# claussss/ubisoft-laforge-daft-exprt

Hardware: AMD Instinct MI355X
Metric: mel frames/sec (fwd+bwd) (higher is better)
Workload: dtype bf16

## Files before the change

include/daft_exprt_hip.h:

```cpp
#ifndef DAFT_EXPRT_HIP_H
#define DAFT_EXPRT_HIP_H

#include <stdint.h>

#ifdef __cplusplus
extern "C" {
#endif

int dx_version(void);
const char* dx_last_error(void);
int dx_prof_enable(int kind, int capacity);
int dx_prof_collect(int kind, int* launches, double* total_ms);

int dx_int_durations(const float* dur, int B, int L, int sampling_rate, int filter_length, int hop_length, int centered,
                     long long* out, long long* totals, int* status);

int dx_pack_dims(int Cout, int Cin, int bf16, int* dims);
int dx_pack_weights(const float* W, void* fwd, void* bwd, int Cout, int Cin, int taps, int bf16, void* stream);
int dx_pack_weights_batched(const void* descs, int n, int bf16, void* stream);
int dx_pack_weights_host(const void* descs, int n, int bf16, void* stream);
int dx_conv_gemm(const void* X, int ldx, const void* Wp, const float* bias, void* Y, int ldy,
                 int B, int N, int Cin, int Cout, int taps, int bf16,
                 int relu, const float* post_scale, const float* post_shift,
                 const void* relu_aux, int ld_aux, int accumulate,
                 const int* lens, int mask_rows, float out_scale, int skip_halo,
                 int x_bf16, int y_bf16, int aux_bf16, const int* rows_exist, void* stream);
int dx_conv_wgrad(const void* dY, int ldy, const void* X, int ldx, float* G,
                  int B, int N, int Cin, int Cout, int taps, const int* lens, int skip_halo,
                  int bf16, int dy_bf16, int x_bf16, float* dbias, void* stream);
typedef struct DxWgradJob {
  const void* dY; const void* X; float* G; float* dbias; const int* lens;
  int ldy, ldx, B, N, Cin, Cout, skip_halo, reserved;
} DxWgradJob;
int dx_conv_wgrad_batched(const void* jobs, int njobs, int taps, int dy_bf16, int x_bf16, void* stream);
int dx_unpack_wgrad(const float* G, float* grad, int Cout, int Cin, int taps, int accumulate, void* stream);
int dx_ff_pair(const void* X, int ldx, const void* Wa, const void* Wb, const float* bias_a, const float* bias_b,
               const void* aux, int ld_aux, void* H, int ldh, float* Y, int ldy,
               int B, int N, int F, int relu_mid, int accumulate, const int* lens, int skip_halo, const int* rows_exist, void* stream);
int dx_ff_pair_ln(const void* X, int ldx, const void* Wa, const void* Wb, const float* bias_a, const float* bias_b, void* H, int ldh, float* Z,
                  int B, int N, int F, const int* lens, int skip_halo, const int* rows_exist,
                  const float* res, const float* ln_w, const float* ln_b, const float* film, int ld_film, float* Yln, float* mean, float* rstd,
                  uint64_t seed_pre, float p_pre, const uint64_t* seed_offset, void* hmask, void* stream);
int dx_ff_pair_ln_qkv(const void* X, int ldx, const void* Wa, const void* Wb, const float* bias_a, const float* bias_b, void* H, int ldh, float* Z,
                      int B, int N, int F, const int* lens, int skip_halo, const int* rows_exist,
                      const float* res, const float* ln_w, const float* ln_b, const float* film, int ld_film, float* Yln, float* mean, float* rstd,
                      uint64_t seed_pre, float p_pre, const uint64_t* seed_offset, const void* Wq, const float* bias_q, void* QKV, void* hmask, void* stream);
int dx_ff_pair_lnbwd(const void* X, int ldx, const void* Wa, const void* Wb, const void* aux, int ld_aux, void* H, int ldh, float* Y,
                     int B, int N, int F, const int* lens, int skip_halo,
                     const float* z, const float* mean, const float* rstd, const float* ln_w, const float* ln_b, void* DG, float* dw, float* db,
                     uint64_t seed_pre, float p_pre, const uint64_t* seed_offset, void* stream);
int dx_ff_block_bwd(const float* dY2, const float* z2, const float* mean2, const float* rstd2, const float* ln2_w, const float* ln2_b,
                    const float* film, int ld_film, void* DG2, float* dw2, float* db2, float* dfilm, int ld_dfilm, uint64_t seed2, float p2,
                    const void* Wa, const void* Wb, const void* aux, int ld_aux, void* H, int ldh, float* Y,
                    int B, int N, int F, const int* lens, int skip_halo,
                    const float* z1, const float* mean1, const float* rstd1, const float* ln1_w, const float* ln1_b, void* DG1, float* dw1, float* db1,
                    uint64_t seed1, float p1, const void* Wout_bwd, void* DATT, const uint64_t* seed_offset, const void* hmask, void* stream);
int dx_colsum(const void* X, int ldx, float* out, long rows, int C, int x_bf16, void* stream);

int dx_length_order(const int* lens, int* order, int B, void* stream);
int dx_attention_fwd(const void* qkv, int ld, const int* lens, void* ctx, int ldc, float* lse,
                     int B, int N, int H, int D, uint64_t seed, const uint64_t* seed_offset, float p_drop, int bf16, int qkv_bf16, int ctx_bf16,
                     const int* order, void* stream);
int dx_attention_proj_ln_fwd(const void* qkv, int ld, const int* lens, void* ctx, int ldc, float* lse, int B, int N, int H, int D,
                             uint64_t seed, const uint64_t* seed_offset, float p_drop,
                             const void* Wpack, const float* proj_bias, float* z, const float* res, const float* w, const float* bias,
                             const float* film, int ld_film, float* y, float* mean, float* rstd, uint64_t seed_pre, float p_pre,
                             void* y_bf16_copy, void* stream);
int dx_attention_bwd(const void* qkv, int ld, const void* ctx, const void* dctx, int ldc, const float* lse, float* delta,
                     const int* lens, void* dqkv, int ldg, int B, int N, int H, int D, uint64_t seed, const uint64_t* seed_offset, float p_drop, int bf16,
                     int qkv_bf16, int dqkv_bf16, int ctx_bf16, const int* order, void* stream);

int dx_ln_fwd(void* a, const void* res, const float* w, const float* bias, const float* film, int ld_film,
              const int* lens, int halo, void* y, float* mean, float* rstd, int B, int N, int C,
              uint64_t seed_pre, float p_pre, uint64_t seed_post, float p_post, const uint64_t* seed_offset, int io_bf16, void* y_bf16_copy,
              void* stream);
int dx_film_affine_fwd(const float* gammas, const float* betas, const float* pm, float* film, int B, int nb, int C, void* stream);
int dx_film_affine_bwd(const void* dfilm_ptrs, const float* gammas, const float* betas, const float* pm, float* dgammas, float* dbetas, float* dpm,
                       int B, int nb, int C, void* stream);
int dx_proj_ln_fwd(const void* X, int ldx, const void* Wpack, const float* proj_bias, float* z, const float* res, const float* w, const float* bias,
                   const float* film, int ld_film, const int* lens, int halo, float* y, float* mean, float* rstd, int B, int N,
                   uint64_t seed_pre, float p_pre, const uint64_t* seed_offset, void* y_bf16_copy, void* stream);
int dx_ln_bwd(const void* dy, const void* z, const float* mean, const float* rstd, const float* w, const float* bias,
              const float* film, int ld_film, const int* lens, int halo, void* dz, void* da, float* dw, float* dbias,
              float* dfilm, int ld_dfilm, int B, int N, int C, int relu_mask,
              uint64_t seed_pre, float p_pre, uint64_t seed_post, float p_post, const uint64_t* seed_offset, int io_bf16, void* dg_bf16_copy,
              void* stream);

int dx_add_pos(const float* x, const long* sym, const float* emb, const float* pe, const int* lens, float* out,
               int B, int N, int D, int pe_rows, void* stream);
int dx_mask_rows(const float* in, const int* lens, float* out, int B, int N, int C, void* stream);
int dx_embedding_bwd(const float* dout, const long* sym, const int* lens, float* demb, int B, int N, int D, void* stream);
int dx_accent_sum(const float* prenet, const float* energy, const float* pitch, const float* we, const float* be,
                  const float* wp, const float* bp, const float* pe, const int* lens, float* out,
                  int B, int N, int D, int pe_rows, void* stream);
int dx_scalar_conv_wgrad(const float* dout, int ldd, const float* rowscale, const float* s0, const float* s1, const int* lens,
                         float* dw0, float* db0, float* dw1, float* db1, int B, int N, int D, void* stream);
int dx_mean_pool(const float* x, const int* lens, float* out, int B, int N, int C, void* stream);
int dx_mean_pool_bwd(const float* dout, const int* lens, float* dx, int B, int N, int C, void* stream);
int dx_transpose(const float* in, float* out, int B, int R, int Cc, int accumulate, void* stream);
int dx_relu_bwd(const float* dy, const float* y, float* out, long n, void* stream);
int dx_channel_affine(const void* x, const float* scale, const float* shift, void* out, long rows, int C, int io_bf16, void* stream);
int dx_l2_normalize(const float* x, float* y, int rows, int C, void* stream);
int dx_cross_entropy(const float* logits, const long* target, float* loss, float* dlogits, int B, int S, void* stream);

int dx_duration_scan(const long* dur_int, float* mu, long* totals, int B, int L, void* stream);
int dx_upsample_prep(const float* enc, const float* dur, const float* energy, const float* pitch,
                     const float* wd, const float* bd, const float* we, const float* be, const float* wp, const float* bp,
                     const float* wr, const float* br, const int* lens, float* xs, float* z, float* sigma,
                     int B, int L, int D, void* stream);
int dx_upsample_fwd(const float* xs, const float* mu, const float* sigma, const int* lens, float* weights, float* xup,
                    int B, int L, int T, int D, void* stream);
int dx_upsample_bwd(const float* dxup, const float* xs, const float* mu, const float* sigma, const float* weights, const int* lens,
                    float* dxs, float* dsigma, int B, int L, int T, int D, void* stream);
int dx_upsample_sym_bwd(const float* dxs_in, const float* dsigma, const float* xs, const float* z, const float* dur, const int* lens,
                        const float* wd, const float* bd, const float* wr, float* dxs_out, float* dz, float* dwr, float* dbr,
                        int B, int L, int D, void* stream);

int dx_mel_stats(const float* mel_pred, const float* mel_target, float* ep, float* et, float* l1sum, float* l2sum,
                 int B, int M, int T, void* stream);
int dx_energy_diff(const float* ep, const float* et, const int* lens, float* des, float* esum, int B, int T, void* stream);
int dx_mel_grad(const float* mel_pred, const float* mel_target, const float* ep, const float* des, const int* lens,
                float c_l1, float c_l2, float c_e, int e_per_total, float* dmel, int B, int M, int T, void* stream);
int dx_loss_finalize(const float* ce, const float* spk_w_dev, float spk_w, const float* dlogits, float* d_spk, int n_logits,
                     const float* pm, float* d_pm, int n_pm, float pmw,
                     const float* l1sum, const float* l2sum, const int* lens, int B, int M, float msw,
                     const float* esum, float ecw, const float* psum, float pcw, float* terms, float* total, float grad_scale, void* stream);
int dx_pitch_mse(const float* pp, int ldp, const float* gt, const int* lens, float* sums, int B, int T, void* stream);
int dx_pitch_grad(const float* pp, int ldp, const float* gt, const int* lens, const float* sums, float scale, float* dpp, int ldd, int B, int T, void* stream);
int dx_pitch_chain_fwd(const float* mel, int B, int M, int T, const int* lens, const void* w0, const void* w1, const void* w2,
                       const float* b0, const float* b1, const float* b2, const float* s0, const float* s1, const float* s2,
                       const float* t0, const float* t1, const float* t2, const float* w3, float b3, float* pp, void* masks, void* stream);
int dx_pitch_chain_bwd(const float* dpp, int B, int M, int T, const int* lens, const void* w0, const void* w1, const void* w2,
                       const float* s0, const float* s1, const float* s2, const float* w3, const void* masks, float* dmel, void* stream);

int dx_condition_prosody(const float* in, float* out, const long* speaker_ids, const float* table, const int* valid,
                         int which, int B, int N, int S, void* stream);
int dx_gather_speaker_rows(const float* emb, const long* speaker_ids, const int* valid, float* out, int B, int E, int S, void* stream);

int dx_sumsq(const float* x, long n, float* out, void* stream);
int dx_adam_step(float* p, const float* g, float* m, float* v, long n, float lr, float beta1, float beta2, float eps,
                 float weight_decay, int step, const float* normsq, float max_norm, float grad_scale, int* skipped,
                 float* norm_out, float* zero_after, void* stream);

#ifdef __cplusplus
}
#endif
#endif
```

ubisoft_laforge_daft_exprt_amd/csrc/dx_f16_names.h:

```cpp
#pragma once
#define dx_accent_sum dx_accent_sum_f16
#define dx_add_pos dx_add_pos_f16
#define dx_attention_bwd dx_attention_bwd_f16
#define dx_attention_fwd dx_attention_fwd_f16
#define dx_attention_proj_ln_fwd dx_attention_proj_ln_fwd_f16
#define dx_channel_affine dx_channel_affine_f16
#define dx_colsum dx_colsum_f16
#define dx_condition_prosody dx_condition_prosody_f16
#define dx_conv_gemm dx_conv_gemm_f16
#define dx_conv_wgrad dx_conv_wgrad_f16
#define dx_conv_wgrad_batched dx_conv_wgrad_batched_f16
#define dx_cross_entropy dx_cross_entropy_f16
#define dx_embedding_bwd dx_embedding_bwd_f16
#define dx_ff_block_bwd dx_ff_block_bwd_f16
#define dx_ff_pair dx_ff_pair_f16
#define dx_ff_pair_ln dx_ff_pair_ln_f16
#define dx_ff_pair_ln_qkv dx_ff_pair_ln_qkv_f16
#define dx_ff_pair_lnbwd dx_ff_pair_lnbwd_f16
#define dx_gather_speaker_rows dx_gather_speaker_rows_f16
#define dx_l2_normalize dx_l2_normalize_f16
#define dx_length_order dx_length_order_f16
#define dx_ln_bwd dx_ln_bwd_f16
#define dx_film_affine_bwd dx_film_affine_bwd_f16
#define dx_film_affine_fwd dx_film_affine_fwd_f16
#define dx_ln_fwd dx_ln_fwd_f16
#define dx_proj_ln_fwd dx_proj_ln_fwd_f16
#define dx_mask_rows dx_mask_rows_f16
#define dx_mean_pool dx_mean_pool_f16
#define dx_mean_pool_bwd dx_mean_pool_bwd_f16
#define dx_pack_dims dx_pack_dims_f16
#define dx_pitch_chain_bwd dx_pitch_chain_bwd_f16
#define dx_pitch_chain_fwd dx_pitch_chain_fwd_f16
#define dx_pack_weights dx_pack_weights_f16
#define dx_pack_weights_batched dx_pack_weights_batched_f16
#define dx_pack_weights_host dx_pack_weights_host_f16
#define dx_relu_bwd dx_relu_bwd_f16
#define dx_scalar_conv_wgrad dx_scalar_conv_wgrad_f16
#define dx_transpose dx_transpose_f16
#define dx_unpack_wgrad dx_unpack_wgrad_f16
```

ubisoft_laforge_daft_exprt_amd/csrc/dx_ffpair.hip:

```cpp
#include "dx_common.h"
#include <algorithm>

namespace {

template <int NJ> struct FP {
  static constexpr int NROW = NJ * 16;
  static constexpr int TOK = NROW - 2;
  static constexpr int HR = NROW + 2;
  static constexpr int IMG = 2 * HR * 128;
  static constexpr int XP = (HR * 16 + 511) / 512;
  static constexpr int RP = (HR + 31) / 32;
};
constexpr int FP_TOK = FP<8>::TOK;

struct FFPairArgs {
  const dx_h16* X; int ldx;
  const dx_h16* Wa; const dx_h16* Wb;
  const float* bias_a; const float* bias_b;
  const dx_h16* aux; int ld_aux;
  dx_h16* H; int ldh;
  float* Y; int ldy;
  int B, N, F;
  int accumulate;
  const int* lens; int skip_halo;
  const int* rows_exist;
  const float* ln_res; const float* ln_w; const float* ln_b; const float* film; int ld_film;
  float* ln_y; float* ln_mean; float* ln_rstd;
  unsigned long long seed_pre; unsigned thresh_pre; float inv_keep_pre; const unsigned long long* seed_offset;
  const dx_h16* q_w; const float* q_bias; dx_h16* q_out;
  const float* lnb_z; const float* lnb_mean; const float* lnb_rstd; const float* lnb_w; const float* lnb_b;
  dx_h16* lnb_dg; float* lnb_dw; float* lnb_db;
  const dx_h16* lnb_wt; dx_h16* lnb_datt;
  const float* lnp_dy; const float* lnp_z; const float* lnp_mean; const float* lnp_rstd; const float* lnp_w; const float* lnp_b;
  const float* lnp_film; int lnp_ld_film;
  dx_h16* lnp_dg; float* lnp_dw; float* lnp_db; float* lnp_dfilm; int lnp_ld_dfilm;
  unsigned long long lnp_seed; unsigned lnp_thresh; float lnp_inv_keep;
  unsigned* hmask;
  unsigned long long* stamps;
};

#ifdef DX_FFPAIR_STAMPS
#define FP_STAMP(K) { if (lane == 0 && wq == 0 && a.stamps) a.stamps[((size_t)blockIdx.x * 2 + role) * 16 + (K)] = __builtin_amdgcn_s_memtime(); }
#else
#define FP_STAMP(K) {}
#endif

__device__ __forceinline__ int fp_lds_off(int row, int slot) { return row * 128 + ((slot ^ (row & 7)) << 4); }

__device__ __forceinline__ uint2 fp_pack4(float a, float b, float c, float d) {
  bf16x4 h;
  h[0] = (dx_h16)a; h[1] = (dx_h16)b; h[2] = (dx_h16)c; h[3] = (dx_h16)d;
  return __builtin_bit_cast(uint2, h);
}

__device__ __forceinline__ int fp_opaque(int x) { asm volatile("" : "+v"(x)); return x; }

__device__ __forceinline__ int fp_wave_sum_i(int v) {
#pragma unroll
  for (int off = 32; off > 0; off >>= 1) v += __shfl_xor(v, off, 64);
  return v;
}

typedef short s16x2 __attribute__((ext_vector_type(2)));

#define FP_MMA(W, X, C) C = DX_MFMA_H16(__builtin_bit_cast(bf16x8, W), __builtin_bit_cast(bf16x8, X), C);

template <bool AUX, bool RELU, int NJ, bool MASK = false>
__global__ __launch_bounds__(512, 2) void ff_pair_kernel(const FFPairArgs a) {
  constexpr int FP_TOK = FP<NJ>::TOK, FP_HR = FP<NJ>::HR, FP_IMG = FP<NJ>::IMG, NROW = FP<NJ>::NROW, XP = FP<NJ>::XP, RP = FP<NJ>::RP;
  extern __shared__ __attribute__((aligned(16))) unsigned char smem[];
  unsigned char* const Xs = smem;
  unsigned char* const Hs0 = smem + FP_IMG;
  unsigned char* const Hs1 = smem + 2 * FP_IMG;
  constexpr int DZ_ROWS = NJ == 8 ? 112 : FP_TOK;
  float* const dzs = a.lnp_w ? reinterpret_cast<float*>(smem + 3 * FP_IMG) : nullptr;

  const int tid = threadIdx.x, lane = tid & 63;
  const int wave = __builtin_amdgcn_readfirstlane(tid >> 6);
  const int role = wave >> 2, wq = wave & 3;
  const int r = lane & 15, g = lane >> 4;
  const int tiles_n = (a.N + FP_TOK - 1) / FP_TOK;
  const int nslices = a.F >> 7;
  FP_STAMP(0)

  const dx_h16* const wbase = role == 0 ? a.Wa + (size_t)(2 * wq) * 4 * 512
                                        : a.Wb + (size_t)(2 * wq) * (a.F >> 5) * 512;
  const unsigned lane16 = lane * 16;
  const int w_tap = role == 0 ? (a.F >> 4) * 4 * 512 : 8 * (a.F >> 5) * 512;
  const int w_i = role == 0 ? 4 * 512 : (a.F >> 5) * 512;
  const int w_slice = role == 0 ? 8 * 4 * 512 : 4 * 512;
  const int total_steps = nslices * 12;
  auto w_ptr = [&](int gs) {
    gs = min(gs, total_steps - 1);
    const int f = fp_opaque(gs / 12), s = gs - f * 12;
    return wbase + (size_t)f * w_slice + (s >> 2) * w_tap + (s & 3) * 512;
  };
  constexpr int RING = NJ == 8 ? 4 : 6;
  f32x4 wr[RING][2];
#define FP_WLOAD(SLOT, GS)                                                                                           \
  {                                                                                                                  \
    const char* p_ = reinterpret_cast<const char*>(w_ptr(GS));                                                       \
    wr[SLOT][0] = *reinterpret_cast<const f32x4*>(p_ + lane16);                                                      \
    wr[SLOT][1] = *reinterpret_cast<const f32x4*>(p_ + (size_t)w_i * 2 + lane16);                                    \
  }

  int b, n0;
  bool live = true;
  if (a.skip_halo >= 0) {
    int nlive = 0;
    int cnt0 = 0, inc0 = 0;
    for (int base = 0; base < a.B; base += 64) {
      const int i = base + lane;
      const int cnt = i < a.B ? min(tiles_n, max(0, (min(a.lens[i] + a.skip_halo, a.N) + FP_TOK - 1) / FP_TOK)) : 0;
      int inc = cnt;
#pragma unroll
      for (int off = 1; off < 64; off <<= 1) { const int v = __shfl_up(inc, off, 64); if (lane >= off) inc += v; }
      if (base == 0) { cnt0 = cnt; inc0 = inc; }
      nlive += __shfl(inc, 63, 64);
    }
    int target = blockIdx.x;
    live = target < nlive;
    if (!live) target -= nlive;
    int run = 0;
    b = 0; n0 = 0;
    for (int base = 0; base < a.B; base += 64) {
      const int i = base + lane;
      int cnt, inc_live;
      if (base == 0) { cnt = cnt0; inc_live = inc0; }
      else {
        cnt = i < a.B ? min(tiles_n, max(0, (min(a.lens[i] + a.skip_halo, a.N) + FP_TOK - 1) / FP_TOK)) : 0;
        inc_live = cnt;
#pragma unroll
        for (int off = 1; off < 64; off <<= 1) { const int v = __shfl_up(inc_live, off, 64); if (lane >= off) inc_live += v; }
      }
      const int rows_here = min(64, a.B - base);
      const int c = live ? cnt : (i < a.B ? tiles_n - cnt : 0);
      const int inc = live ? inc_live : min(lane + 1, rows_here) * tiles_n - inc_live;
      const unsigned long long hit = __ballot(target < run + inc);
      if (hit) {
        const int first = __builtin_ctzll(hit);
        const int excl = __shfl(run + inc - c, first, 64), cnt_b = __shfl(cnt, first, 64);
        b = base + first;
        n0 = (live ? target - excl : cnt_b + (target - excl)) * FP_TOK;
        break;
      }
      run += __shfl(inc, 63, 64);
    }
  } else {
    b = blockIdx.x / tiles_n;
    n0 = (blockIdx.x - b * tiles_n) * FP_TOK;
  }
  FP_STAMP(1)
  b = __builtin_amdgcn_readfirstlane(b);
  n0 = __builtin_amdgcn_readfirstlane(n0);

  if (!live) {
    const int rows = min(FP_TOK, a.N - n0);
    const int hu = a.H ? a.F >> 3 : 0;
    for (int u = tid; u < rows * hu; u += 512) {
      const int row = u / hu, q = u - row * hu;
      *reinterpret_cast<f32x4*>(a.H + ((size_t)b * a.N + n0 + row) * a.ldh + q * 8) = f32x4{0.f, 0.f, 0.f, 0.f};
    }
    if (a.lnb_w)
      for (int u = tid; u < rows * 16; u += 512) {
        const int row = u >> 4, q = u & 15;
        *reinterpret_cast<f32x4*>(a.lnb_dg + ((size_t)b * a.N + n0 + row) * 128 + q * 8) = f32x4{0.f, 0.f, 0.f, 0.f};
        if (a.lnp_w) *reinterpret_cast<f32x4*>(a.lnp_dg + ((size_t)b * a.N + n0 + row) * 128 + q * 8) = f32x4{0.f, 0.f, 0.f, 0.f};
        if (a.lnb_wt) *reinterpret_cast<f32x4*>(a.lnb_datt + ((size_t)b * a.N + n0 + row) * 128 + q * 8) = f32x4{0.f, 0.f, 0.f, 0.f};
      }
    if (a.lnp_w)
      for (int u = tid; u < rows * 32; u += 512) {
        const int row = u >> 5, q = u & 31;
        *reinterpret_cast<f32x4*>(a.Y + ((size_t)b * a.N + n0 + row) * a.ldy + q * 4) = f32x4{0.f, 0.f, 0.f, 0.f};
      }
    if (!a.accumulate)
      for (int u = tid; u < rows * 32; u += 512) {
        const int row = u >> 5, q = u & 31;
        *reinterpret_cast<f32x4*>(a.Y + ((size_t)b * a.N + n0 + row) * a.ldy + q * 4) = f32x4{0.f, 0.f, 0.f, 0.f};
        if (a.ln_w) *reinterpret_cast<f32x4*>(a.ln_y + ((size_t)b * a.N + n0 + row) * 128 + q * 4) = f32x4{0.f, 0.f, 0.f, 0.f};
      }
    if (a.q_w)
      for (int u = tid; u < rows * 48; u += 512) {
        const int row = u / 48, q = u - row * 48;
        *reinterpret_cast<f32x4*>(a.q_out + ((size_t)b * a.N + n0 + row) * 384 + q * 8) = f32x4{0.f, 0.f, 0.f, 0.f};
      }
    return;
  }

  const int NL = a.rows_exist ? a.rows_exist[b] : a.N;
  if (a.lnp_w) {
    const int q = tid & 15;
    const int len_b = a.lens ? a.lens[b] : a.N;
    float wv[8], bv[8], fg[8];
#pragma unroll
    for (int e = 0; e < 8; ++e) {
      wv[e] = a.lnp_w[q * 8 + e]; bv[e] = a.lnp_b[q * 8 + e];
      fg[e] = a.lnp_film ? a.lnp_film[(size_t)b * a.lnp_ld_film + q * 8 + e] : 1.f;
    }
    const unsigned long long seed = a.lnp_seed + (a.seed_offset ? *a.seed_offset : 0ull);
    float gw[8], gb[8], gfg[8], gfb[8];
#pragma unroll
    for (int e = 0; e < 8; ++e) gw[e] = gb[e] = gfg[e] = gfb[e] = 0.f;
    f32x4 dyv[RP][2], zv[RP][2];
    float muv[RP], rsv[RP];
#pragma unroll
    for (int it = 0; it < RP; ++it) {
      const int row = (tid >> 4) + it * 32, n = n0 - 2 + row;
      const bool valid = row < FP_HR && n >= 0 && n < len_b && n < NL;
      const size_t grow = (size_t)b * a.N + n;
#pragma unroll
      for (int hh = 0; hh < 2; ++hh) {
        dyv[it][hh] = valid ? *reinterpret_cast<const f32x4*>(a.lnp_dy + grow * 128 + q * 8 + hh * 4) : f32x4{0.f, 0.f, 0.f, 0.f};
        zv[it][hh] = valid ? *reinterpret_cast<const f32x4*>(a.lnp_z + grow * 128 + q * 8 + hh * 4) : f32x4{0.f, 0.f, 0.f, 0.f};
      }
      muv[it] = valid ? a.lnp_mean[grow] : 0.f;
      rsv[it] = valid ? a.lnp_rstd[grow] : 0.f;
    }
    FP_WLOAD(0, 0) FP_WLOAD(1, 1) FP_WLOAD(2, 2) FP_WLOAD(3, 3)
    if constexpr (RING == 6) { FP_WLOAD(4, 4) FP_WLOAD(5, 5) }
#pragma unroll
    for (int it = 0; it < RP; ++it) {
      const int row = (tid >> 4) + it * 32, n = n0 - 2 + row;
      const bool inb = row < FP_HR && n >= 0 && n < a.N;
      const bool owned = inb && row >= 2 && row < 2 + FP_TOK;
      const bool ownvalid = owned && n < len_b;
      const size_t grow = (size_t)b * a.N + n;
      float dz[8];
      float s1 = 0.f, s2 = 0.f, g[8], xh[8];
#pragma unroll
      for (int e = 0; e < 8; ++e) {
        const float z = zv[it][e >> 2][e & 3];
        float d = dyv[it][e >> 2][e & 3];
        xh[e] = (z - muv[it]) * rsv[it];
        const float ln = xh[e] * wv[e] + bv[e];
        if (ownvalid) { gfg[e] += d * ln; gfb[e] += d; }
        d *= fg[e];
        if (ownvalid) { gw[e] += d * xh[e]; gb[e] += d; }
        g[e] = d * wv[e];
        s1 += g[e]; s2 += g[e] * xh[e];
      }
#pragma unroll
      for (int off = 1; off < 16; off <<= 1) { s1 += __shfl_xor(s1, off, 64); s2 += __shfl_xor(s2, off, 64); }
      s1 *= (1.0f / 128); s2 *= (1.0f / 128);
#pragma unroll
      for (int e = 0; e < 8; ++e) dz[e] = rsv[it] * (g[e] - s1 - xh[e] * s2);
      if (owned) {
        if (dzs && row - 2 < DZ_ROWS) {
          *reinterpret_cast<f32x4*>(dzs + (row - 2) * 128 + q * 8) = f32x4{dz[0], dz[1], dz[2], dz[3]};
          *reinterpret_cast<f32x4*>(dzs + (row - 2) * 128 + q * 8 + 4) = f32x4{dz[4], dz[5], dz[6], dz[7]};
        } else {
          *reinterpret_cast<f32x4*>(a.Y + grow * a.ldy + q * 8) = f32x4{dz[0], dz[1], dz[2], dz[3]};
          *reinterpret_cast<f32x4*>(a.Y + grow * a.ldy + q * 8 + 4) = f32x4{dz[4], dz[5], dz[6], dz[7]};
        }
      }
      if (a.lnp_thresh) {
        float f[8];
        dx_dropout_scale4(seed, (unsigned long long)grow * 128 + q * 8, a.lnp_thresh, a.lnp_inv_keep, f);
        dx_dropout_scale4(seed, (unsigned long long)grow * 128 + q * 8 + 4, a.lnp_thresh, a.lnp_inv_keep, f + 4);
#pragma unroll
        for (int e = 0; e < 8; ++e) dz[e] *= f[e];
      }
      bf16x8 h8;
#pragma unroll
      for (int e = 0; e < 8; ++e) h8[e] = (dx_h16)dz[e];
      const f32x4 hv = __builtin_bit_cast(f32x4, h8);
      if (owned) *reinterpret_cast<f32x4*>(a.lnp_dg + grow * 128 + q * 8) = hv;
      if (row < FP_HR) *reinterpret_cast<f32x4*>(Xs + (q >> 3) * (FP_HR * 128) + fp_lds_off(row, q & 7)) = hv;
    }
#pragma unroll
    for (int e = 0; e < 8; ++e) {
#pragma unroll
      for (int off = 16; off < 64; off <<= 1) {
        gw[e] += __shfl_xor(gw[e], off, 64); gb[e] += __shfl_xor(gb[e], off, 64);
        gfg[e] += __shfl_xor(gfg[e], off, 64); gfb[e] += __shfl_xor(gfb[e], off, 64);
      }
    }
    float* const red = reinterpret_cast<float*>(Hs0);
    if (lane < 16) {
#pragma unroll
      for (int e = 0; e < 8; ++e) {
        red[(wave * 4 + 0) * 128 + q * 8 + e] = gw[e]; red[(wave * 4 + 1) * 128 + q * 8 + e] = gb[e];
        red[(wave * 4 + 2) * 128 + q * 8 + e] = gfg[e]; red[(wave * 4 + 3) * 128 + q * 8 + e] = gfb[e];
      }
    }
    __syncthreads();
    {
      const int quant = tid >> 7, c = tid & 127;
      float t = 0.f;
#pragma unroll
      for (int w8 = 0; w8 < 8; ++w8) t += red[(w8 * 4 + quant) * 128 + c];
      if (t != 0.f) {
        if (quant == 0) atomicAdd(&a.lnp_dw[c], t);
        else if (quant == 1) atomicAdd(&a.lnp_db[c], t);
        else if (a.lnp_dfilm) atomicAdd(&a.lnp_dfilm[(size_t)b * a.lnp_ld_dfilm + (quant == 3 ? 128 : 0) + c], t);
      }
    }
    __syncthreads();
    if (tid < 64) {
      const int img = tid >> 5, rr = NROW + ((tid >> 4) & 1), qq = tid & 15;
      *reinterpret_cast<f32x4*>((img ? Hs1 : Hs0) + (qq >> 3) * (FP_HR * 128) + fp_lds_off(rr, qq & 7)) = f32x4{0.f, 0.f, 0.f, 0.f};
    }
  } else
  {
    f32x4 xr[XP];
#pragma unroll
    for (int it = 0; it < XP; ++it) {
      const int u = tid + it * 512;
      const int row = u >> 4, q = u & 15;
      const int n = n0 - 2 + row;
      f32x4 v = f32x4{0.f, 0.f, 0.f, 0.f};
      if (u < FP_HR * 16 && n >= 0 && n < NL) v = *reinterpret_cast<const f32x4*>(a.X + ((size_t)b * a.N + n) * a.ldx + q * 8);
      xr[it] = v;
    }
    FP_WLOAD(0, 0) FP_WLOAD(1, 1) FP_WLOAD(2, 2) FP_WLOAD(3, 3)
    if constexpr (RING == 6) { FP_WLOAD(4, 4) FP_WLOAD(5, 5) }
    if (tid < 64) {
      const int img = tid >> 5, rr = NROW + ((tid >> 4) & 1), q = tid & 15;
      *reinterpret_cast<f32x4*>((img ? Hs1 : Hs0) + (q >> 3) * (FP_HR * 128) + fp_lds_off(rr, q & 7)) = f32x4{0.f, 0.f, 0.f, 0.f};
    }
#pragma unroll
    for (int it = 0; it < XP; ++it) {
      const int u = tid + it * 512;
      const int row = u >> 4, q = u & 15;
      if (u < FP_HR * 16) *reinterpret_cast<f32x4*>(Xs + (q >> 3) * (FP_HR * 128) + fp_lds_off(row, q & 7)) = xr[it];
    }
  }
  __syncthreads();
  FP_STAMP(2)

  int foff[3][2];
#pragma unroll
  for (int t = 0; t < 3; ++t)
#pragma unroll
    for (int hh = 0; hh < 2; ++hh) foff[t][hh] = fp_lds_off(r + t, hh * 4 + g);
  const int len_cols = min(FP_TOK, a.N - n0);
  const int h_rows = a.H ? len_cols : 0;

#define FP_CO_RD(K, IMGC)                                                                                            \
  {                                                                                                                  \
    const int u_ = fp_opaque(tid) + NROW * 8 + (K) * 256;        \
    const int row_ = u_ >> 4, q_ = u_ & 15;                                                                          \
    cpv = *reinterpret_cast<const f32x4*>((IMGC) + (q_ >> 3) * (FP_HR * 128) + fp_lds_off(min(row_, NROW - 1) + 1, q_ & 7)); \
  }
#define FP_CO_ST(K, F0C)                                                                                             \
  {                                                                                                                  \
    const int u_ = fp_opaque(tid) + NROW * 8 + (K) * 256;                                                            \
    const int row_ = u_ >> 4, q_ = u_ & 15;                                                                          \
    if (row_ < h_rows) *reinterpret_cast<f32x4*>(a.H + ((size_t)b * a.N + n0 + row_) * a.ldh + (F0C) + q_ * 8) = cpv; \
  }
#define FP_COPY_OUT_CONS(IMGC, F0C)                                                                                  \
  {                                                                                                                  \
    f32x4 cv_[NJ / 2];                                                                                               \
    const int t_ = fp_opaque(tid) - 256;                        \
    _Pragma("unroll") for (int k = 0; k < NJ / 2; ++k) {                                                                  \
      const int u_ = t_ + k * 256;                                                                                   \
      cv_[k] = *reinterpret_cast<const f32x4*>((IMGC) + ((u_ & 15) >> 3) * (FP_HR * 128) + fp_lds_off((u_ >> 4) + 1, u_ & 7)); \
    }                                                                                                                \
    _Pragma("unroll") for (int k = 0; k < NJ / 2; ++k) {                                                             \
      const int u_ = t_ + k * 256;                                                                                   \
      const int row_ = u_ >> 4, q_ = u_ & 15;                                                                        \
      if (row_ < h_rows) *reinterpret_cast<f32x4*>(a.H + ((size_t)b * a.N + n0 + row_) * a.ldh + (F0C) + q_ * 8) = cv_[k]; \
    }                                                                                                                \
  }

#define FP_RD8(DST, IMG, S)                                                                                          \
  {                                                                                                                  \
    const unsigned char* const bp_ = (IMG) + (((S) & 3) >> 1) * (FP_HR * 128) + foff[((S) >> 2) % 3][(S) & 1];       \
    _Pragma("unroll") for (int j = 0; j < NJ; ++j) DST[j] = *reinterpret_cast<const float4*>(bp_ + j * 2048);        \
  }
#define FP_STEP(CUR, NXT, IMG, GS0, S, AUXPF, FRESH, CO, IMGC, F0C)                                                  \
  {                                                                                                                  \
    if ((S) + 1 < 12) FP_RD8(NXT, IMG, (S) + 1)                                                                      \
    if ((CO) && (S) < NJ && ((S) & 1) == 0) FP_CO_RD((S) >> 1, IMGC)                                                 \
    __builtin_amdgcn_sched_barrier(0);                                                                               \
    const f32x4 w0 = wr[(S) % RING][0], w1 = wr[(S) % RING][1];                                                      \
    if ((FRESH) && (S) == 0) {                                   \
      _Pragma("unroll") for (int j = 0; j < NJ; ++j) { acc[0][j] = bv0; FP_MMA(w0, CUR[j], acc[0][j]) }              \
      _Pragma("unroll") for (int j = 0; j < NJ; ++j) { acc[1][j] = bv1; FP_MMA(w1, CUR[j], acc[1][j]) }              \
    } else {                                                                                                         \
      _Pragma("unroll") for (int j = 0; j < NJ; ++j) { FP_MMA(w0, CUR[j], acc[0][j]) }                               \
      _Pragma("unroll") for (int j = 0; j < NJ; ++j) { FP_MMA(w1, CUR[j], acc[1][j]) }                               \
    }                                                                                                                \
    FP_WLOAD((S) % RING, (GS0) + (S) + RING)                                                                         \
    if ((CO) && (S) < NJ && ((S) & 1) == 1) FP_CO_ST((S) >> 1, F0C)                                                  \
    if ((S) == 8) { AUXPF }                                                                                          \
    __builtin_amdgcn_sched_barrier(0);                                                                               \
  }
#define FP_SLICE_STEPS(IMG, GS0, AUXPF, FR, CO, IMGC, F0C)                                                           \
  {                                                                                                                  \
    float4 xa[NJ], xb[NJ];                                                                                           \
    f32x4 cpv;                                                                                                       \
    FP_RD8(xa, IMG, 0)                                                                                               \
    FP_STEP(xa, xb, IMG, GS0, 0, AUXPF, FR, CO, IMGC, F0C) FP_STEP(xb, xa, IMG, GS0, 1, AUXPF, FR, CO, IMGC, F0C)    \
    FP_STEP(xa, xb, IMG, GS0, 2, AUXPF, FR, CO, IMGC, F0C) FP_STEP(xb, xa, IMG, GS0, 3, AUXPF, FR, CO, IMGC, F0C)    \
    FP_STEP(xa, xb, IMG, GS0, 4, AUXPF, FR, CO, IMGC, F0C) FP_STEP(xb, xa, IMG, GS0, 5, AUXPF, FR, CO, IMGC, F0C)    \
    FP_STEP(xa, xb, IMG, GS0, 6, AUXPF, FR, CO, IMGC, F0C) FP_STEP(xb, xa, IMG, GS0, 7, AUXPF, FR, CO, IMGC, F0C)    \
    FP_STEP(xa, xb, IMG, GS0, 8, AUXPF, FR, CO, IMGC, F0C) FP_STEP(xb, xa, IMG, GS0, 9, AUXPF, FR, CO, IMGC, F0C)    \
    FP_STEP(xa, xb, IMG, GS0, 10, AUXPF, FR, CO, IMGC, F0C) FP_STEP(xb, xa, IMG, GS0, 11, AUXPF, FR, CO, IMGC, F0C)  \
  }

  unsigned char* const stage = smem;
  if (role == 0) {
    f32x4 acc[2][NJ];
    const bool edge = n0 == 0 || n0 + FP_TOK >= NL;
    const int tile_lin = b * tiles_n + n0 / FP_TOK;
#define FP_PRODUCE(F_, COFLAG)                                                                                       \
    {                                                                                                                \
      const int f0 = (F_) << 7;                                                                                      \
                                   \
      const f32x4 bv0 = a.bias_a ? *reinterpret_cast<const f32x4*>(a.bias_a + f0 + 32 * wq + 4 * g) : f32x4{0.f, 0.f, 0.f, 0.f};      \
      const f32x4 bv1 = a.bias_a ? *reinterpret_cast<const f32x4*>(a.bias_a + f0 + 32 * wq + 16 + 4 * g) : f32x4{0.f, 0.f, 0.f, 0.f}; \
      bf16x4 av[2][MASK ? 1 : NJ];                                                                                   \
      unsigned mw[2] = {0u, 0u};                                                                                     \
      FP_SLICE_STEPS(Xs, (F_) * 12,                                                                                  \
        if constexpr (AUX) {                                                                                         \
          if constexpr (MASK) {                                                                                      \
            const unsigned* mp_ = a.hmask + ((((size_t)tile_lin * nslices + (f0 >> 7)) * 4 + wq) * 2) * 64 + fp_opaque(lane); \
            mw[0] = mp_[0]; mw[1] = mp_[64];                                                                         \
          } else {                                                                                                   \
          const int r2_ = fp_opaque(r);                                                                              \
          const int g2_ = fp_opaque(g);                                                                              \
          _Pragma("unroll") for (int i = 0; i < 2; ++i)                                                              \
            _Pragma("unroll") for (int j = 0; j < NJ; ++j) {                                                         \
              const int n = min(max(n0 - 1 + 16 * j + r2_, 0), a.N - 1);                                             \
              av[i][j] = *reinterpret_cast<const bf16x4*>(a.aux + ((size_t)b * a.N + n) * a.ld_aux + f0 + 32 * wq + 16 * i + 4 * g2_); \
            }                                                                                                        \
          }                                                                                                          \
        }, true, COFLAG, ((((F_) - 1) & 1) ? Hs1 : Hs0), ((F_) - 1) * 128)                                           \
      unsigned char* const out = ((F_) & 1) ? Hs1 : Hs0;                                                             \
      const int r_ = fp_opaque(r);                                                                                   \
      const int g_ = fp_opaque(g);                                                                                   \
      _Pragma("unroll") for (int i = 0; i < 2; ++i) {                                                                \
        const int c = 32 * wq + 16 * i + 4 * g_;                                                                     \
        unsigned char* const orow = out + (c >> 6) * (FP_HR * 128) + fp_lds_off(r_, (c & 63) >> 3) + ((g_ & 1) << 3); \
        unsigned sw_ = 0u;                                                  \
        const unsigned mwi_ = mw[i];                                                                                 \
        _Pragma("unroll") for (int j = 0; j < NJ; ++j) {                                                             \
          f32x4 v = acc[i][j];                                                                                       \
          if constexpr (AUX) {                                                                                       \
            if constexpr (MASK) {                                                                                    \
               \
              _Pragma("unroll") for (int e = 0; e < 4; ++e) {                                                        \
                const float ve_ = v[e];                                                                              \
                const unsigned ke_ = __float_as_uint(ve_) & (unsigned)__builtin_amdgcn_sbfe((int)mwi_, NJ * 4 - 1 - (j * 4 + e), 1); \
                v[e] = __uint_as_float(ke_);                                                                         \
              }                                                                                                      \
            } else {                                                                                                 \
              _Pragma("unroll") for (int e = 0; e < 4; ++e) if (!((float)av[i][j][e] > 0.f)) v[e] = 0.f;             \
            }                                                                                                        \
          }                                                                                                          \
          if (edge) { const int n = n0 - 1 + 16 * j + r_; if (n < 0 || n >= NL) v = f32x4{0.f, 0.f, 0.f, 0.f}; }    \
          if constexpr (RELU) {                                                                                      \
             \
            if (a.hmask) {                                                                                           \
              _Pragma("unroll") for (int e = 0; e < 4; ++e) {                                                        \
                const float ve_ = v[e];                                                                              \
                sw_ = __builtin_amdgcn_alignbit(sw_, __float_as_uint(ve_) - 1u, 31);                                 \
              }                                                                                                      \
            }                                                                                                        \
          }                                                                                                          \
          uint2 pk = fp_pack4(v[0], v[1], v[2], v[3]);                                                               \
          if constexpr (RELU) {                                                                                      \
             \
            pk.x = __builtin_bit_cast(unsigned, __builtin_elementwise_max(__builtin_bit_cast(s16x2, pk.x), s16x2{0, 0})); \
            pk.y = __builtin_bit_cast(unsigned, __builtin_elementwise_max(__builtin_bit_cast(s16x2, pk.y), s16x2{0, 0})); \
          }                                                                                                          \
          *reinterpret_cast<uint2*>(orow + j * 2048) = pk;                                                           \
        }                                                                                                            \
        if constexpr (RELU) {                                        \
          if (a.hmask) a.hmask[((((size_t)tile_lin * nslices + (f0 >> 7)) * 4 + wq) * 2 + i) * 64 + fp_opaque(lane)] = ~sw_; \
        }                                                                                                            \
      }                                                                                                              \
    }
    FP_PRODUCE(0, false)
    __syncthreads();
    FP_STAMP(3)
    for (int it = 1; it < nslices; ++it) {
      if (it == 4) FP_STAMP(12)
      FP_PRODUCE(it, true)
      if (it == 4) FP_STAMP(14)
      __syncthreads();
      FP_STAMP(3 + it)
    }
    {
      const unsigned char* const imgc = ((nslices - 1) & 1) ? Hs1 : Hs0;
      f32x4 cpv;
#pragma unroll
      for (int k = 0; k < NJ / 2; ++k) { FP_CO_RD(k, imgc) FP_CO_ST(k, (nslices - 1) << 7) }
    }
    __syncthreads();
    FP_STAMP(3 + nslices)
#undef FP_PRODUCE
  } else {
    f32x4 acc[2][NJ];
    const f32x4 bv0 = f32x4{0.f, 0.f, 0.f, 0.f}, bv1 = bv0;
#pragma unroll
    for (int i = 0; i < 2; ++i)
#pragma unroll
      for (int j = 0; j < NJ; ++j) acc[i][j] = f32x4{0.f, 0.f, 0.f, 0.f};
    __syncthreads();
    FP_STAMP(3)
    for (int it = 1; it <= nslices; ++it) {
      if (it == 4) FP_STAMP(12)
      const int f = it - 1;
      const unsigned char* const img = (f & 1) ? Hs1 : Hs0;
      FP_COPY_OUT_CONS(img, f << 7)
      FP_SLICE_STEPS(img, f * 12, , false, false, img, 0)
      if (it == 4) FP_STAMP(13)
      __syncthreads();
      FP_STAMP(3 + it)
    }
#pragma unroll
    for (int i = 0; i < 2; ++i) {
      const int co = 32 * wq + 16 * i + 4 * g;
      const f32x4 bv = a.bias_b ? *reinterpret_cast<const f32x4*>(a.bias_b + co) : f32x4{0.f, 0.f, 0.f, 0.f};
#pragma unroll
      for (int j = 0; j < NJ; ++j) {
        const int q = 16 * j + r;
        *reinterpret_cast<f32x4*>(stage + q * 512 + (((co >> 2) ^ (q & 15)) << 4)) = acc[i][j] + bv;
      }
    }
  }
#undef FP_SLICE_STEPS
#undef FP_STEP
#undef FP_RD8
#undef FP_COPY_OUT_CONS
#undef FP_CO_RD
#undef FP_CO_ST

  __syncthreads();
  if (a.ln_w) {
    const int s = tid & 31;
    const f32x4 wv = *reinterpret_cast<const f32x4*>(a.ln_w + s * 4), bv = *reinterpret_cast<const f32x4*>(a.ln_b + s * 4);
    f32x4 fg = f32x4{1.f, 1.f, 1.f, 1.f}, fb = f32x4{0.f, 0.f, 0.f, 0.f};
    if (a.film) {
      fg = *reinterpret_cast<const f32x4*>(a.film + (size_t)b * a.ld_film + s * 4);
      fb = *reinterpret_cast<const f32x4*>(a.film + (size_t)b * a.ld_film + 128 + s * 4);
    }
    const int len_b = a.lens ? a.lens[b] : a.N;
    const unsigned long long seed = a.seed_pre + (a.seed_offset ? *a.seed_offset : 0ull);
    bf16x8 qa[3][4];
    if (a.q_w) {
#pragma unroll
      for (int i = 0; i < 3; ++i)
#pragma unroll
        for (int ks = 0; ks < 4; ++ks) qa[i][ks] = *reinterpret_cast<const bf16x8*>(a.q_w + (size_t)((wave * 3 + i) * 4 + ks) * 512 + lane * 8);
    }
    f32x4 resv[NJ];
#pragma unroll
    for (int k = 0; k < NJ; ++k) {
      const int row = (tid >> 5) + k * 16, n = n0 + row;
      resv[k] = (row < len_cols && n < len_b) ? *reinterpret_cast<const f32x4*>(a.ln_res + ((size_t)b * a.N + n) * 128 + s * 4) : f32x4{0.f, 0.f, 0.f, 0.f};
    }
#pragma unroll
    for (int k = 0; k < NJ; ++k) {
      const int row = (tid >> 5) + k * 16, n = n0 + row;
      const bool inb = row < len_cols, valid = inb && n < len_b;
      const size_t grow = (size_t)b * a.N + n;
      f32x4 z = f32x4{0.f, 0.f, 0.f, 0.f};
      if (valid) {
        z = *reinterpret_cast<const f32x4*>(stage + row * 512 + ((s ^ (row & 15)) << 4));
        if (a.thresh_pre) {
          float f[4];
          dx_dropout_scale4(seed, (unsigned long long)grow * 128 + s * 4, a.thresh_pre, a.inv_keep_pre, f);
          z[0] *= f[0]; z[1] *= f[1]; z[2] *= f[2]; z[3] *= f[3];
        }
        z += resv[k];
      }
      if (inb) *reinterpret_cast<f32x4*>(a.Y + grow * a.ldy + s * 4) = z;
      float sum = (z[0] + z[1]) + (z[2] + z[3]);
#pragma unroll
      for (int off = 1; off < 32; off <<= 1) sum += __shfl_xor(sum, off, 64);
      const float mu = sum * (1.0f / 128);
      const f32x4 d = z - mu;
      float q = (d[0] * d[0] + d[1] * d[1]) + (d[2] * d[2] + d[3] * d[3]);
#pragma unroll
      for (int off = 1; off < 32; off <<= 1) q += __shfl_xor(q, off, 64);
      const float rs = 1.0f / sqrtf(q * (1.0f / 128) + 1e-5f);
      if (inb && s == 0) { a.ln_mean[grow] = valid ? mu : 0.f; a.ln_rstd[grow] = valid ? rs : 0.f; }
      f32x4 y = d * rs * wv + bv;
      if (a.film) y = fg * y + fb;
      if (!valid) y = f32x4{0.f, 0.f, 0.f, 0.f};
      if (inb) *reinterpret_cast<f32x4*>(a.ln_y + grow * 128 + s * 4) = y;
      if (a.q_w) {
        bf16x4 h4;
        h4[0] = (dx_h16)y[0]; h4[1] = (dx_h16)y[1]; h4[2] = (dx_h16)y[2]; h4[3] = (dx_h16)y[3];
        *reinterpret_cast<bf16x4*>(stage + row * 512 + (((s >> 1) ^ (row & 15)) << 4) + ((s & 1) << 3)) = h4;
      }
    }
    if (a.q_w) {
      __syncthreads();
      f32x4 qb[3];
#pragma unroll
      for (int i = 0; i < 3; ++i) qb[i] = *reinterpret_cast<const f32x4*>(a.q_bias + (wave * 3 + i) * 16 + g * 4);
#pragma unroll 2
      for (int j = 0; j < NJ; ++j) {
        const int row = j * 16 + r;
        bf16x8 xb[4];
#pragma unroll
        for (int ks = 0; ks < 4; ++ks) xb[ks] = *reinterpret_cast<const bf16x8*>(stage + row * 512 + (((ks * 4 + g) ^ (row & 15)) << 4));
        f32x4 acc[3];
#pragma unroll
        for (int i = 0; i < 3; ++i) acc[i] = qb[i];
#pragma unroll
        for (int ks = 0; ks < 4; ++ks)
#pragma unroll
          for (int i = 0; i < 3; ++i) acc[i] = DX_MFMA_H16(qa[i][ks], xb[ks], acc[i]);
        if (row < len_cols) {
          dx_h16* const orow = a.q_out + ((size_t)b * a.N + n0 + row) * 384 + wave * 48 + g * 4;
#pragma unroll
          for (int i = 0; i < 3; ++i) {
            bf16x4 o4;
            o4[0] = (dx_h16)acc[i][0]; o4[1] = (dx_h16)acc[i][1]; o4[2] = (dx_h16)acc[i][2]; o4[3] = (dx_h16)acc[i][3];
            *reinterpret_cast<bf16x4*>(orow + i * 16) = o4;
          }
        }
      }
    }
  } else if (a.lnb_w) {
    const int s = tid & 31;
    const f32x4 wv = *reinterpret_cast<const f32x4*>(a.lnb_w + s * 4), bv = *reinterpret_cast<const f32x4*>(a.lnb_b + s * 4);
    (void)bv;
    const int len_b = a.lens ? a.lens[b] : a.N;
    const unsigned long long seed = a.seed_pre + (a.seed_offset ? *a.seed_offset : 0ull);
    f32x4 oldv[NJ], zv[NJ];
    float muv[NJ], rsv[NJ];
#pragma unroll
    for (int k = 0; k < NJ; ++k) {
      const int row = (tid >> 5) + k * 16, n = n0 + row;
      const bool valid = row < len_cols && n < len_b;
      const size_t grow = (size_t)b * a.N + n;
      if (dzs && row < DZ_ROWS) oldv[k] = valid ? *reinterpret_cast<const f32x4*>(dzs + row * 128 + s * 4) : f32x4{0.f, 0.f, 0.f, 0.f};
      else oldv[k] = valid ? *reinterpret_cast<const f32x4*>(a.Y + grow * a.ldy + s * 4) : f32x4{0.f, 0.f, 0.f, 0.f};
      zv[k] = valid ? *reinterpret_cast<const f32x4*>(a.lnb_z + grow * 128 + s * 4) : f32x4{0.f, 0.f, 0.f, 0.f};
      muv[k] = valid ? a.lnb_mean[grow] : 0.f;
      rsv[k] = valid ? a.lnb_rstd[grow] : 0.f;
    }
    f32x4 gw = f32x4{0.f, 0.f, 0.f, 0.f}, gb = gw;
#pragma unroll
    for (int k = 0; k < NJ; ++k) {
      const int row = (tid >> 5) + k * 16, n = n0 + row;
      const bool inb = row < len_cols, valid = inb && n < len_b;
      const size_t grow = (size_t)b * a.N + n;
      f32x4 d = f32x4{0.f, 0.f, 0.f, 0.f};
      if (valid) d = *reinterpret_cast<const f32x4*>(stage + row * 512 + ((s ^ (row & 15)) << 4)) + oldv[k];
      const f32x4 xh = (zv[k] - muv[k]) * rsv[k];
      gw += d * xh; gb += d;
      const f32x4 g = d * wv;
      float s1 = (g[0] + g[1]) + (g[2] + g[3]);
      const f32x4 gx = g * xh;
      float s2 = (gx[0] + gx[1]) + (gx[2] + gx[3]);
#pragma unroll
      for (int off = 1; off < 32; off <<= 1) { s1 += __shfl_xor(s1, off, 64); s2 += __shfl_xor(s2, off, 64); }
      s1 *= (1.0f / 128); s2 *= (1.0f / 128);
      f32x4 dz = (g - s1 - xh * s2) * rsv[k];
      if (!inb) continue;
      *reinterpret_cast<f32x4*>(a.Y + grow * a.ldy + s * 4) = dz;
      if (a.thresh_pre) {
        float f[4];
        dx_dropout_scale4(seed, (unsigned long long)grow * 128 + s * 4, a.thresh_pre, a.inv_keep_pre, f);
        dz[0] *= f[0]; dz[1] *= f[1]; dz[2] *= f[2]; dz[3] *= f[3];
      }
      bf16x4 h4;
      h4[0] = (dx_h16)dz[0]; h4[1] = (dx_h16)dz[1]; h4[2] = (dx_h16)dz[2]; h4[3] = (dx_h16)dz[3];
      *reinterpret_cast<bf16x4*>(a.lnb_dg + grow * 128 + s * 4) = h4;
      if (a.lnb_wt) *reinterpret_cast<bf16x4*>(stage + row * 512 + (((s >> 1) ^ (row & 15)) << 4) + ((s & 1) << 3)) = h4;
    }
    if (a.lnb_wt) {
#pragma unroll
      for (int k = 0; k < NJ; ++k) {
        const int row = (tid >> 5) + k * 16;
        if (row >= len_cols) *reinterpret_cast<uint2*>(stage + row * 512 + (((s >> 1) ^ (row & 15)) << 4) + ((s & 1) << 3)) = make_uint2(0u, 0u);
      }
    }
    float* const red = reinterpret_cast<float*>(smem + NROW * 512);
    *reinterpret_cast<f32x4*>(red + (tid >> 5) * 128 + s * 4) = gw;
    *reinterpret_cast<f32x4*>(red + 2048 + (tid >> 5) * 128 + s * 4) = gb;
    __syncthreads();
    if (tid < 256) {
      const float* src = red + (tid >> 7) * 2048 + (tid & 127);
      float t = 0.f;
#pragma unroll
      for (int q = 0; q < 16; ++q) t += src[q * 128];
      if (t != 0.f) atomicAdd((tid >> 7) ? &a.lnb_db[tid & 127] : &a.lnb_dw[tid & 127], t);
    }
    if (a.lnb_wt) {
      constexpr int CB = NJ;
      const int rb = wave % NJ, cb0 = (wave / NJ) * CB;
      const int row = rb * 16 + r;
      bf16x8 xb[4];
#pragma unroll
      for (int ks = 0; ks < 4; ++ks) xb[ks] = *reinterpret_cast<const bf16x8*>(stage + row * 512 + (((ks * 4 + g) ^ (row & 15)) << 4));
      f32x4 acc[CB];
#pragma unroll
      for (int i = 0; i < CB; ++i) acc[i] = f32x4{0.f, 0.f, 0.f, 0.f};
#pragma unroll
      for (int ks = 0; ks < 4; ++ks) {
        bf16x8 wa[CB];
#pragma unroll
        for (int i = 0; i < CB; ++i) wa[i] = *reinterpret_cast<const bf16x8*>(a.lnb_wt + (size_t)((cb0 + i) * 4 + ks) * 512 + lane * 8);
#pragma unroll
        for (int i = 0; i < CB; ++i) acc[i] = DX_MFMA_H16(wa[i], xb[ks], acc[i]);
      }
      if (row < len_cols) {
        dx_h16* const orow = a.lnb_datt + ((size_t)b * a.N + n0 + row) * 128 + cb0 * 16 + g * 4;
#pragma unroll
        for (int i = 0; i < CB; ++i) {
          bf16x4 o4;
          o4[0] = (dx_h16)acc[i][0]; o4[1] = (dx_h16)acc[i][1]; o4[2] = (dx_h16)acc[i][2]; o4[3] = (dx_h16)acc[i][3];
          *reinterpret_cast<bf16x4*>(orow + i * 16) = o4;
        }
      }
    }
  } else {
    f32x4 old[NJ];
    if (a.accumulate) {
#pragma unroll
      for (int k = 0; k < NJ; ++k) {
        const int u = tid + k * 512;
        const int row = min(u >> 5, len_cols - 1), s = u & 31;
        old[k] = *reinterpret_cast<const f32x4*>(a.Y + ((size_t)b * a.N + n0 + row) * a.ldy + s * 4);
      }
    }
#pragma unroll
    for (int k = 0; k < NJ; ++k) {
      const int u = tid + k * 512;
      const int row = u >> 5, s = u & 31;
      f32x4 v = *reinterpret_cast<const f32x4*>(stage + row * 512 + ((s ^ (row & 15)) << 4));
      if (a.accumulate) v += old[k];
      if (row < len_cols) *reinterpret_cast<f32x4*>(a.Y + ((size_t)b * a.N + n0 + row) * a.ldy + s * 4) = v;
    }
  }
  FP_STAMP(15)
#undef FP_WLOAD
}

#undef FP_MMA

}

#ifdef DX_FFPAIR_STAMPS
static unsigned long long* g_ffpair_stamps = nullptr;
extern "C" void dx_ff_pair_set_stamps(unsigned long long* p) { g_ffpair_stamps = p; }
#endif

extern "C" {

static int ff_pair_launch(const void* X, int ldx, const void* Wa, const void* Wb, const float* bias_a, const float* bias_b,
                          const void* aux, int ld_aux, void* H, int ldh, float* Y, int ldy,
                          int B, int N, int F, int relu_mid, int accumulate, const int* lens, int skip_halo, const int* rows_exist,
                          const float* ln_res, const float* ln_w, const float* ln_b, const float* film, int ld_film,
                          float* ln_y, float* ln_mean, float* ln_rstd, unsigned long long seed_pre, float p_pre, const unsigned long long* seed_offset,
                          const float* lnb_z, const float* lnb_mean, const float* lnb_rstd, const float* lnb_w, const float* lnb_b,
                          void* lnb_dg, float* lnb_dw, float* lnb_db, const FFPairArgs* prologue, void* stream, unsigned* hmask = nullptr) {
  DX_REQUIRE((X || prologue) && Wa && Wb && Y, "dx_ff_pair: null pointer");
  DX_REQUIRE(H || (relu_mid && !lnb_w), "dx_ff_pair: only the forward pair may omit the mid-activation output H");
  if (ln_w) {
    DX_REQUIRE(relu_mid && !accumulate && lens && skip_halo >= 0 && ldy == 128, "dx_ff_pair_ln: forward pair, no accumulate, lens, dense Z");
    DX_REQUIRE(ln_res && ln_b && ln_y && ln_mean && ln_rstd, "dx_ff_pair_ln: null pointer");
    DX_REQUIRE(!film || ld_film >= 256, "dx_ff_pair_ln: ld_film too small");
    DX_REQUIRE(p_pre >= 0.f && p_pre < 1.f, "dx_ff_pair_ln: dropout p out of range");
  }
  if (lnb_w) {
    DX_REQUIRE(aux && accumulate && lens && skip_halo >= 0 && ldy == 128 && !ln_w, "dx_ff_pair_lnbwd: input-gradient pair accumulating onto a dense Y, lens required");
    DX_REQUIRE(lnb_z && lnb_mean && lnb_rstd && lnb_b && lnb_dg && lnb_dw && lnb_db, "dx_ff_pair_lnbwd: null pointer");
    DX_REQUIRE(p_pre >= 0.f && p_pre < 1.f && ((uintptr_t)lnb_dg % 16) == 0, "dx_ff_pair_lnbwd: bad dropout p or alignment");
  }
  DX_REQUIRE(B > 0 && N > 0 && F >= 128 && (F % 128) == 0, "dx_ff_pair: bad dims B=%d N=%d F=%d (F must be a multiple of 128)", B, N, F);
  DX_REQUIRE(ldx >= 128 && (ldx % 8) == 0 && ldh >= F && (ldh % 8) == 0 && ldy >= 128 && (ldy % 4) == 0, "dx_ff_pair: bad leading dimensions");
  DX_REQUIRE(!aux || (ld_aux >= F && (ld_aux % 4) == 0), "dx_ff_pair: bad ld_aux");
  DX_REQUIRE((aux != nullptr) != (relu_mid != 0), "dx_ff_pair: exactly one of relu_mid (forward) and aux (backward) must be given");
  DX_REQUIRE(skip_halo < 0 || lens, "dx_ff_pair: skip_halo needs lens");
  if (prologue && prologue->q_w) {
    DX_REQUIRE(ln_w && prologue->q_bias && prologue->q_out && ((uintptr_t)prologue->q_w % 16) == 0 && ((uintptr_t)prologue->q_out % 16) == 0,
               "dx_ff_pair_ln_qkv: needs the LayerNorm epilogue, a bias and 16-byte aligned pointers");
  } else if (prologue) {
    DX_REQUIRE(lnb_w && prologue->lnp_dy && prologue->lnp_z && prologue->lnp_mean && prologue->lnp_rstd && prologue->lnp_w && prologue->lnp_b &&
               prologue->lnp_dg && prologue->lnp_dw && prologue->lnp_db, "dx_ff_block_bwd: null pointer");
    DX_REQUIRE((prologue->lnp_film == nullptr) == (prologue->lnp_dfilm == nullptr), "dx_ff_block_bwd: film and dfilm must come together");
    DX_REQUIRE(((uintptr_t)prologue->lnp_dy % 16) == 0 && ((uintptr_t)prologue->lnp_z % 16) == 0 && ((uintptr_t)prologue->lnp_dg % 16) == 0,
               "dx_ff_block_bwd: pointers must be 16-byte aligned");
  }
  DX_REQUIRE(((uintptr_t)X % 16) == 0 && ((uintptr_t)Wa % 16) == 0 && ((uintptr_t)Wb % 16) == 0 && ((uintptr_t)H % 16) == 0 &&
             ((uintptr_t)Y % 16) == 0 && ((uintptr_t)aux % 8) == 0, "dx_ff_pair: pointers must be 16-byte aligned");
  FFPairArgs a{(const dx_h16*)X, ldx, (const dx_h16*)Wa, (const dx_h16*)Wb, bias_a, bias_b, (const dx_h16*)aux, ld_aux,
               (dx_h16*)H, ldh, Y, ldy, B, N, F, accumulate, lens, skip_halo, rows_exist,
               ln_res, ln_w, ln_b, film, ld_film, ln_y, ln_mean, ln_rstd, seed_pre, (unsigned)lrintf(p_pre * 65536.f), 1.f / (1.f - p_pre), seed_offset,
               nullptr, nullptr, nullptr,
               lnb_z, lnb_mean, lnb_rstd, lnb_w, lnb_b, (dx_h16*)lnb_dg, lnb_dw, lnb_db};
  if (prologue && prologue->q_w) { a.q_w = prologue->q_w; a.q_bias = prologue->q_bias; a.q_out = prologue->q_out; }
  if (prologue && prologue->lnp_dy) {
    a.lnp_dy = prologue->lnp_dy; a.lnp_z = prologue->lnp_z; a.lnp_mean = prologue->lnp_mean; a.lnp_rstd = prologue->lnp_rstd;
    a.lnp_w = prologue->lnp_w; a.lnp_b = prologue->lnp_b; a.lnp_film = prologue->lnp_film; a.lnp_ld_film = prologue->lnp_ld_film;
    a.lnp_dg = prologue->lnp_dg; a.lnp_dw = prologue->lnp_dw; a.lnp_db = prologue->lnp_db; a.lnp_dfilm = prologue->lnp_dfilm;
    a.lnp_ld_dfilm = prologue->lnp_ld_dfilm; a.lnp_seed = prologue->lnp_seed; a.lnp_thresh = prologue->lnp_thresh; a.lnp_inv_keep = prologue->lnp_inv_keep;
    a.lnb_wt = prologue->lnb_wt; a.lnb_datt = prologue->lnb_datt;
  }
#ifdef DX_FFPAIR_STAMPS
  a.stamps = g_ffpair_stamps;
#endif
  constexpr int DZ8 = 112 * 512, DZ4 = FP<4>::TOK * 512;
  const int lds8 = 3 * FP<8>::IMG + (a.lnp_w ? DZ8 : 0), lds4 = 3 * FP<4>::IMG + (a.lnp_w ? DZ4 : 0);
  static bool configured = false;
  if (!configured) {
    hipFuncSetAttribute(reinterpret_cast<const void*>(&ff_pair_kernel<true, false, 8>), hipFuncAttributeMaxDynamicSharedMemorySize, 3 * FP<8>::IMG + DZ8);
    hipFuncSetAttribute(reinterpret_cast<const void*>(&ff_pair_kernel<true, false, 8, true>), hipFuncAttributeMaxDynamicSharedMemorySize, 3 * FP<8>::IMG + DZ8);
    hipFuncSetAttribute(reinterpret_cast<const void*>(&ff_pair_kernel<true, false, 4, true>), hipFuncAttributeMaxDynamicSharedMemorySize, 3 * FP<4>::IMG + DZ4);
    hipFuncSetAttribute(reinterpret_cast<const void*>(&ff_pair_kernel<false, true, 8>), hipFuncAttributeMaxDynamicSharedMemorySize, 3 * FP<8>::IMG);
    hipFuncSetAttribute(reinterpret_cast<const void*>(&ff_pair_kernel<true, false, 4>), hipFuncAttributeMaxDynamicSharedMemorySize, 3 * FP<4>::IMG + DZ4);
    hipFuncSetAttribute(reinterpret_cast<const void*>(&ff_pair_kernel<false, true, 4>), hipFuncAttributeMaxDynamicSharedMemorySize, 3 * FP<4>::IMG);
    configured = true;
  }
  a.hmask = hmask;
  const int nj = B * dx_cdiv(N, FP<8>::TOK) >= 96 ? 8 : 4;
  hipStream_t s = (hipStream_t)stream;
  dx_prof_begin(DX_PROF_CONV_GEMM, s);
  if (nj == 8) {
    if (aux && hmask) hipLaunchKernelGGL((ff_pair_kernel<true, false, 8, true>), dim3(B * dx_cdiv(N, FP<8>::TOK)), dim3(512), lds8, s, a);
    else if (aux) hipLaunchKernelGGL((ff_pair_kernel<true, false, 8>), dim3(B * dx_cdiv(N, FP<8>::TOK)), dim3(512), lds8, s, a);
    else hipLaunchKernelGGL((ff_pair_kernel<false, true, 8>), dim3(B * dx_cdiv(N, FP<8>::TOK)), dim3(512), 3 * FP<8>::IMG, s, a);
  } else {
    if (aux && hmask) hipLaunchKernelGGL((ff_pair_kernel<true, false, 4, true>), dim3(B * dx_cdiv(N, FP<4>::TOK)), dim3(512), lds4, s, a);
    else if (aux) hipLaunchKernelGGL((ff_pair_kernel<true, false, 4>), dim3(B * dx_cdiv(N, FP<4>::TOK)), dim3(512), lds4, s, a);
    else hipLaunchKernelGGL((ff_pair_kernel<false, true, 4>), dim3(B * dx_cdiv(N, FP<4>::TOK)), dim3(512), 3 * FP<4>::IMG, s, a);
  }
  dx_prof_end(DX_PROF_CONV_GEMM, s);
  DX_LAUNCH_CHECK("dx_ff_pair");
  return DX_OK;
}

int dx_ff_pair(const void* X, int ldx, const void* Wa, const void* Wb, const float* bias_a, const float* bias_b,
               const void* aux, int ld_aux, void* H, int ldh, float* Y, int ldy,
               int B, int N, int F, int relu_mid, int accumulate, const int* lens, int skip_halo, const int* rows_exist, void* stream) {
  return ff_pair_launch(X, ldx, Wa, Wb, bias_a, bias_b, aux, ld_aux, H, ldh, Y, ldy, B, N, F, relu_mid, accumulate, lens, skip_halo, rows_exist,
                        nullptr, nullptr, nullptr, nullptr, 0, nullptr, nullptr, nullptr, 0ull, 0.f, nullptr,
                        nullptr, nullptr, nullptr, nullptr, nullptr, nullptr, nullptr, nullptr, nullptr, stream);
}

int dx_ff_pair_ln(const void* X, int ldx, const void* Wa, const void* Wb, const float* bias_a, const float* bias_b, void* H, int ldh, float* Z,
                  int B, int N, int F, const int* lens, int skip_halo, const int* rows_exist,
                  const float* res, const float* ln_w, const float* ln_b, const float* film, int ld_film, float* Yln, float* mean, float* rstd,
                  uint64_t seed_pre, float p_pre, const uint64_t* seed_offset, void* hmask, void* stream) {
  DX_REQUIRE(ln_w != nullptr, "dx_ff_pair_ln: null pointer");
  return ff_pair_launch(X, ldx, Wa, Wb, bias_a, bias_b, nullptr, 0, H, ldh, Z, 128, B, N, F, 1, 0, lens, skip_halo, rows_exist,
                        res, ln_w, ln_b, film, ld_film, Yln, mean, rstd, (unsigned long long)seed_pre, p_pre, (const unsigned long long*)seed_offset,
                        nullptr, nullptr, nullptr, nullptr, nullptr, nullptr, nullptr, nullptr, nullptr, stream, (unsigned*)hmask);
}

int dx_ff_pair_ln_qkv(const void* X, int ldx, const void* Wa, const void* Wb, const float* bias_a, const float* bias_b, void* H, int ldh, float* Z,
                      int B, int N, int F, const int* lens, int skip_halo, const int* rows_exist,
                      const float* res, const float* ln_w, const float* ln_b, const float* film, int ld_film, float* Yln, float* mean, float* rstd,
                      uint64_t seed_pre, float p_pre, const uint64_t* seed_offset, const void* Wq, const float* bias_q, void* QKV, void* hmask, void* stream) {
  DX_REQUIRE(ln_w != nullptr && Wq != nullptr, "dx_ff_pair_ln_qkv: null pointer");
  FFPairArgs ext{};
  ext.q_w = (const dx_h16*)Wq; ext.q_bias = bias_q; ext.q_out = (dx_h16*)QKV;
  return ff_pair_launch(X, ldx, Wa, Wb, bias_a, bias_b, nullptr, 0, H, ldh, Z, 128, B, N, F, 1, 0, lens, skip_halo, rows_exist,
                        res, ln_w, ln_b, film, ld_film, Yln, mean, rstd, (unsigned long long)seed_pre, p_pre, (const unsigned long long*)seed_offset,
                        nullptr, nullptr, nullptr, nullptr, nullptr, nullptr, nullptr, nullptr, &ext, stream, (unsigned*)hmask);
}

int dx_ff_pair_lnbwd(const void* X, int ldx, const void* Wa, const void* Wb, const void* aux, int ld_aux, void* H, int ldh, float* Y,
                     int B, int N, int F, const int* lens, int skip_halo,
                     const float* z, const float* mean, const float* rstd, const float* ln_w, const float* ln_b, void* DG, float* dw, float* db,
                     uint64_t seed_pre, float p_pre, const uint64_t* seed_offset, void* stream) {
  DX_REQUIRE(ln_w != nullptr, "dx_ff_pair_lnbwd: null pointer");
  return ff_pair_launch(X, ldx, Wa, Wb, nullptr, nullptr, aux, ld_aux, H, ldh, Y, 128, B, N, F, 0, 1, lens, skip_halo, nullptr,
                        nullptr, nullptr, nullptr, nullptr, 0, nullptr, nullptr, nullptr, (unsigned long long)seed_pre, p_pre, (const unsigned long long*)seed_offset,
                        z, mean, rstd, ln_w, ln_b, DG, dw, db, nullptr, stream);
}

int dx_ff_block_bwd(const float* dY2, const float* z2, const float* mean2, const float* rstd2, const float* ln2_w, const float* ln2_b,
                    const float* film, int ld_film, void* DG2, float* dw2, float* db2, float* dfilm, int ld_dfilm, uint64_t seed2, float p2,
                    const void* Wa, const void* Wb, const void* aux, int ld_aux, void* H, int ldh, float* Y,
                    int B, int N, int F, const int* lens, int skip_halo,
                    const float* z1, const float* mean1, const float* rstd1, const float* ln1_w, const float* ln1_b, void* DG1, float* dw1, float* db1,
                    uint64_t seed1, float p1, const void* Wout_bwd, void* DATT, const uint64_t* seed_offset, const void* hmask, void* stream) {
  DX_REQUIRE(ln1_w != nullptr && ln2_w != nullptr, "dx_ff_block_bwd: null pointer");
  DX_REQUIRE((Wout_bwd == nullptr) == (DATT == nullptr) && ((uintptr_t)Wout_bwd % 16) == 0 && ((uintptr_t)DATT % 16) == 0, "dx_ff_block_bwd: Wout_bwd and DATT come together, 16-byte aligned");
  DX_REQUIRE(p2 >= 0.f && p2 < 1.f, "dx_ff_block_bwd: dropout p out of range");
  DX_REQUIRE(!film || (ld_film >= 256 && ld_dfilm >= 256), "dx_ff_block_bwd: ld_film / ld_dfilm too small");
  FFPairArgs pro{};
  pro.lnp_dy = dY2; pro.lnp_z = z2; pro.lnp_mean = mean2; pro.lnp_rstd = rstd2; pro.lnp_w = ln2_w; pro.lnp_b = ln2_b;
  pro.lnp_film = film; pro.lnp_ld_film = ld_film; pro.lnp_dg = (dx_h16*)DG2; pro.lnp_dw = dw2; pro.lnp_db = db2; pro.lnp_dfilm = dfilm;
  pro.lnb_wt = (const dx_h16*)Wout_bwd; pro.lnb_datt = (dx_h16*)DATT;
  pro.lnp_ld_dfilm = ld_dfilm; pro.lnp_seed = (unsigned long long)seed2; pro.lnp_thresh = (unsigned)lrintf(p2 * 65536.f); pro.lnp_inv_keep = 1.f / (1.f - p2);
  return ff_pair_launch(nullptr, 128, Wa, Wb, nullptr, nullptr, aux, ld_aux, H, ldh, Y, 128, B, N, F, 0, 1, lens, skip_halo, nullptr,
                        nullptr, nullptr, nullptr, nullptr, 0, nullptr, nullptr, nullptr, (unsigned long long)seed1, p1, (const unsigned long long*)seed_offset,
                        z1, mean1, rstd1, ln1_w, ln1_b, DG1, dw1, db1, &pro, stream, (unsigned*)hmask);
}

}
```

ubisoft_laforge_daft_exprt_amd/ops.py:

```python
from __future__ import annotations

import ctypes

import torch

from . import _lib
from ._lib import lib

PRECISIONS = ('f32', 'bf16', 'fp16')


class Runtime:

    def __init__(self, precision='f32'):
        self.precision = _check_precision(precision)
        self.pack_epoch = 0
        self.sink = False
        self.launch_log = None
        self.arena = None
        self.arena_hint = 1 << 20
        self.seed_offset = None
        self.defer_wgrad = False
        self.wgrad_queue = {}
        self.backward_split = None
        self.cut_levels = 0
        self._packs = []
        self._tables = {}

    def set_precision(self, name):
        self.precision = _check_precision(name)

    def __deepcopy__(self, memo):
        new = Runtime(self.precision)
        new.pack_epoch = self.pack_epoch
        memo[id(self)] = new
        return new

    def invalidate_packs(self):
        self.pack_epoch += 1

    def record_launches(self, enable: bool):
        log = self.launch_log
        self.launch_log = [] if enable else None
        return log


def _check_precision(name):
    if name not in PRECISIONS:
        raise ValueError(f"precision must be one of {PRECISIONS}, got {name!r}")
    return name


DEFAULT = Runtime('f32')


def set_precision(name: str) -> None:
    DEFAULT.set_precision(name)


def get_precision() -> str:
    return DEFAULT.precision


def invalidate_packs(rt=None) -> None:
    (rt or DEFAULT).invalidate_packs()


def record_launches(enable: bool, rt=None):
    return (rt or DEFAULT).record_launches(enable)


def _half(prec) -> int:
    return 1 if prec in ('bf16', 'fp16') else 0


_H16 = {'bf16': torch.bfloat16, 'fp16': torch.float16}


def _fn(name, prec):
    return getattr(lib(), name + '_f16' if prec == 'fp16' else name)


def _p(t):
    return None if t is None else t.data_ptr()


def _stream():
    return torch.cuda.current_stream().cuda_stream


def _chk(t, name):
    if not t.is_cuda or t.dtype not in (torch.float32, torch.bfloat16, torch.float16):
        raise TypeError(f'{name} must be a float32 (or, in a 16-bit operand mode, bfloat16 / float16) tensor on the GPU (got {t.dtype} on {t.device})')
    return t


def _is_bf16(t):
    return int(t is not None and t.dtype in (torch.bfloat16, torch.float16))


def _check_h16(prec, *tensors):
    want = _H16.get(prec)
    for t in tensors:
        if t is not None and t.dtype in (torch.bfloat16, torch.float16) and t.dtype != want:
            raise TypeError(f'{t.dtype} tensor in {prec!r} operand mode')


def hidden_dtype(prec=None):
    return _H16.get(prec or DEFAULT.precision, torch.float32)


def _rows(t):
    if t.stride(-1) != 1:
        raise ValueError('last dimension must be contiguous')
    ld = t.stride(-2)
    if t.dim() == 3 and t.stride(0) != t.shape[1] * ld:
        raise ValueError('batch rows must be densely stacked')
    return ld


def repack_all(rt=None, packs=None) -> int:
    import struct
    rt = rt or DEFAULT
    prec = rt.precision
    live = [r() for r in rt._packs] if packs is None else list(packs)
    stale = []
    for pk in live:
        if pk is None or not pk.weight.is_cuda:
            continue
        img = pk._image(prec)
        if pk._current_key() != img.key:
            stale.append((pk, img))
    if not stale:
        return 0
    sig = (prec,) + tuple((pk.weight.data_ptr(), img.fwd.data_ptr(), img.bwd.data_ptr()) for pk, img in stale)
    table = rt._tables.get(sig)
    if table is None:
        recs = b''.join(struct.pack('<QQQ8i', pk.weight.data_ptr(), img.fwd.data_ptr(), img.bwd.data_ptr(), pk.cout, pk.cin, pk.taps,
                                     img.dims[0], img.dims[1], img.dims[2], img.dims[3], 0) for pk, img in stale)
        table = ctypes.create_string_buffer(recs, len(recs))
        if len(rt._tables) > 8:
            rt._tables.clear()
        rt._tables[sig] = table
    _fn('dx_pack_weights_host', prec)(ctypes.addressof(table), len(stale), _half(prec), _stream())
    for pk, img in stale:
        img.key = pk._current_key()
    return len(stale)


class _PackImage:
    __slots__ = ('fwd', 'bwd', 'dims', 'key', 'half')

    def __init__(self):
        self.fwd = self.bwd = self.dims = self.key = None
        self.half = 0


class PackedWeight:

    def __init__(self, weight: torch.Tensor, rt: Runtime = None):
        import weakref
        self.weight = weight
        self.rt = rt or DEFAULT
        self.cout, self.cin = weight.shape[0], weight.shape[1]
        self.taps = weight.shape[2] if weight.dim() == 3 else 1
        self._images = {}
        self.rt._packs.append(weakref.ref(self))
        if len(self.rt._packs) > 4096:
            self.rt._packs[:] = [r for r in self.rt._packs if r() is not None]

    def __deepcopy__(self, memo):
        import copy
        new = PackedWeight(copy.deepcopy(self.weight, memo), copy.deepcopy(self.rt, memo))
        memo[id(self)] = new
        return new

    def _current_key(self):
        w = self.weight
        return (w._version, w.data_ptr(), self.rt.pack_epoch if w.requires_grad else 0)

    def _image(self, prec) -> _PackImage:
        img = self._images.get(prec)
        w = self.weight
        if img is None or img.fwd.device != w.device:
            img = _PackImage()
            img.half = _half(prec)
            dt = _H16.get(prec, torch.float32)
            dims = (ctypes.c_int * 4)()
            lib().dx_pack_dims(self.cout, self.cin, img.half, ctypes.cast(dims, ctypes.c_void_p))
            img.dims = [int(d) for d in dims]
            img.fwd = torch.empty(self.taps * img.dims[0] * img.dims[1], dtype=dt, device=w.device)
            img.bwd = torch.empty(self.taps * img.dims[2] * img.dims[3], dtype=dt, device=w.device)
            self._images[prec] = img
        return img

    def image(self, prec=None) -> _PackImage:
        prec = prec or self.rt.precision
        img = self._image(prec)
        key = self._current_key()
        if key != img.key:
            _fn('dx_pack_weights', prec)(_p(self.weight.detach()), _p(img.fwd), _p(img.bwd), self.cout, self.cin, self.taps, img.half, _stream())
            img.key = key
        return img

    def refresh(self, prec=None):
        self.image(prec)
        return self


def _log(pack_or_rt, rec):
    rt = pack_or_rt.rt if isinstance(pack_or_rt, PackedWeight) else (pack_or_rt or DEFAULT)
    if rt.launch_log is not None:
        rt.launch_log.append(rec)


def conv_gemm(x, pack: PackedWeight, bias=None, *, transpose=False, relu=False, post_scale=None, post_shift=None,
              relu_aux=None, out=None, accumulate=False, lens=None, mask_rows=False, out_scale=1.0, B=None, N=None, halo=-1,
              out_dtype=torch.float32, prec=None, rows_exist=None):
    _chk(x, 'x')
    prec = prec or pack.rt.precision
    _check_h16(prec, x, out, relu_aux)
    img = pack.image(prec)
    if x.dim() == 2:
        B_, N_ = (1, x.shape[0]) if B is None else (B, N)
    else:
        B_, N_ = x.shape[0], x.shape[1]
    cin, cout = (pack.cout, pack.cin) if transpose else (pack.cin, pack.cout)
    if x.shape[-1] != cin:
        raise ValueError(f'expected {cin} input channels, got {x.shape[-1]}')
    ldx = _rows(x)
    if out is None:
        out = torch.empty(*x.shape[:-1], cout, dtype=out_dtype, device=x.device)
    ldy = _rows(out)
    _log(pack, ('conv', B_ * N_, N_, cin, cout, pack.taps))
    _fn('dx_conv_gemm', prec)(_p(x), ldx, _p(img.bwd if transpose else img.fwd), _p(bias), _p(out), ldy, B_, N_, cin, cout, pack.taps,
                       img.half, int(relu), _p(post_scale), _p(post_shift), _p(relu_aux),
                       0 if relu_aux is None else _rows(relu_aux), int(accumulate), _p(lens), int(mask_rows), float(out_scale), int(halo),
                       _is_bf16(x), _is_bf16(out), _is_bf16(relu_aux), _p(rows_exist), _stream())
    return out


_FF_FUSED_MIN_TILES = 96
_FF_FUSED_MIN_TILES62 = 64


def ff_pair_applies(x, pack1: PackedWeight, pack2: PackedWeight, prec) -> bool:
    return (prec in _H16 and x.dtype == _H16[prec] and x.dim() == 3 and x.shape[2] == 128 and pack1.taps == 3 and pack2.taps == 3
            and pack1.cin == 128 and pack2.cout == 128 and pack2.cin == pack1.cout and pack1.cout % 128 == 0
            and (x.shape[0] * ((x.shape[1] + 125) // 126) >= _FF_FUSED_MIN_TILES or x.shape[0] * ((x.shape[1] + 61) // 62) >= _FF_FUSED_MIN_TILES62))


def ff_pair(x, pack1: PackedWeight, pack2: PackedWeight, bias1, bias2, lens, *, backward=False, aux=None, out=None, accumulate=False,
            halo=1, prec=None, rows_exist=None):
    prec = pack1.rt.precision if prec is None else prec
    if prec not in _H16 or x.dtype != _H16[prec]:
        raise TypeError('ff_pair runs in a 16-bit operand mode on an activation tensor of that type')
    B, N, D = x.shape
    Fc = pack1.cout
    if D != 128 or pack1.cin != 128 or pack2.cout != 128 or pack2.cin != Fc or pack1.taps != 3 or pack2.taps != 3:
        raise ValueError('ff_pair is built for conv(k=3, 128 -> F) -> conv(k=3, F -> 128)')
    i1, i2 = pack1.image(prec), pack2.image(prec)
    wa, wb = (i2.bwd, i1.bwd) if backward else (i1.fwd, i2.fwd)
    h = torch.empty(B, N, Fc, dtype=_H16[prec], device=x.device)
    if out is None:
        out = torch.empty(B, N, 128, dtype=torch.float32, device=x.device)
    _log(pack1, ('ffpair', B * N, N, 128, Fc, 3))
    _fn('dx_ff_pair', prec)(_p(x), _rows(x), _p(wa), _p(wb), _p(bias1), _p(bias2), _p(aux), 0 if aux is None else _rows(aux), _p(h), _rows(h),
                     _p(out), _rows(out), B, N, Fc, int(not backward), int(accumulate), _p(lens), int(halo), _p(rows_exist), _stream())
    return out, h


def next_qkv_applies(pack_in: PackedWeight, prec) -> bool:
    return _half(prec) == 1 and pack_in.taps == 1 and pack_in.cin == 128 and pack_in.cout == 384


def ff_pair_ln(x, pack1: PackedWeight, pack2: PackedWeight, bias1, bias2, lens, res, ln_w, ln_b, film, *, seed_pre=0, p_pre=0.0, seed_offset=None,
               halo=1, prec=None, rows_exist=None, next_in=None, need_h=True, want_mask=False):
    prec = pack1.rt.precision if prec is None else prec
    B, N, D = x.shape
    Fc = pack1.cout
    i1, i2 = pack1.image(prec), pack2.image(prec)
    h = torch.empty(B, N, Fc, dtype=_H16[prec], device=x.device) if need_h else None
    z = torch.empty(B, N, 128, dtype=torch.float32, device=x.device)
    y = torch.empty_like(z)
    mean = torch.empty(B, N, dtype=torch.float32, device=x.device)
    rstd = torch.empty(B, N, dtype=torch.float32, device=x.device)
    mask = torch.empty(B * ((N + 61) // 62), Fc // 128, 4, 2, 64, dtype=torch.int32, device=x.device) if want_mask else None
    tail = (mask,) if want_mask else ()
    _log(pack1, ('ffpair', B * N, N, 128, Fc, 3))
    if next_in is not None:
        pq, bq = next_in
        qkv = torch.empty(B, N, 384, dtype=_H16[prec], device=x.device)
        _log(pq, ('conv', B * N, N, 128, 384, 1))
        _fn('dx_ff_pair_ln_qkv', prec)(_p(x), _rows(x), _p(i1.fwd), _p(i2.fwd), _p(bias1), _p(bias2), _p(h), Fc if h is None else _rows(h), _p(z), B, N, Fc, _p(lens), int(halo),
                                       _p(rows_exist), _p(res), _p(ln_w), _p(ln_b), _p(film), 0 if film is None else film.stride(0), _p(y), _p(mean),
                                       _p(rstd), seed_pre, float(p_pre), _p(seed_offset), _p(pq.image(prec).fwd), _p(bq), _p(qkv), _p(mask), _stream())
        return (z, h, y, mean, rstd, qkv) + tail
    _fn('dx_ff_pair_ln', prec)(_p(x), _rows(x), _p(i1.fwd), _p(i2.fwd), _p(bias1), _p(bias2), _p(h), Fc if h is None else _rows(h), _p(z), B, N, Fc, _p(lens), int(halo),
                               _p(rows_exist), _p(res), _p(ln_w), _p(ln_b), _p(film), 0 if film is None else film.stride(0), _p(y), _p(mean), _p(rstd),
                               seed_pre, float(p_pre), _p(seed_offset), _p(mask), _stream())
    return (z, h, y, mean, rstd) + tail




def ff_pair_lnbwd(x, pack1: PackedWeight, pack2: PackedWeight, lens, aux, out, z, mean, rstd, ln_w, ln_b, *, seed_pre=0, p_pre=0.0, seed_offset=None,
                  halo=1, prec=None, arena=None, w_sink=None, b_sink=None):
    prec = pack1.rt.precision if prec is None else prec
    B, N, D = x.shape
    Fc = pack1.cout
    i1, i2 = pack1.image(prec), pack2.image(prec)
    dh = torch.empty(B, N, Fc, dtype=_H16[prec], device=x.device)
    dg = torch.empty(B, N, 128, dtype=_H16[prec], device=x.device)
    dw = w_sink if w_sink is not None else _zeros(arena, 128, device=x.device)
    db = b_sink if b_sink is not None else _zeros(arena, 128, device=x.device)
    _log(pack1, ('ffpair', B * N, N, 128, Fc, 3))
    _fn('dx_ff_pair_lnbwd', prec)(_p(x), _rows(x), _p(i2.bwd), _p(i1.bwd), _p(aux), _rows(aux), _p(dh), _rows(dh), _p(out), B, N, Fc, _p(lens), int(halo),
                                  _p(z), _p(mean), _p(rstd), _p(ln_w), _p(ln_b), _p(dg), _p(dw), _p(db), seed_pre, float(p_pre), _p(seed_offset), _stream())
    return out, dh, dg, (None if w_sink is not None else dw), (None if b_sink is not None else db)


def ff_block_bwd(dy2, z2, mean2, rstd2, ln2_w, ln2_b, film, pack1: PackedWeight, pack2: PackedWeight, lens, aux, z1, mean1, rstd1, ln1_w, ln1_b, *,
                 seed2=0, p2=0.0, seed1=0, p1=0.0, seed_offset=None, halo=1, prec=None, arena=None, sinks=None, out_pack=None, hmask=None):
    prec = pack1.rt.precision if prec is None else prec
    B, N, D = dy2.shape
    Fc = pack1.cout
    dev = dy2.device
    sinks = sinks or {}
    i1, i2 = pack1.image(prec), pack2.image(prec)
    dz1 = torch.empty(B, N, 128, dtype=torch.float32, device=dev)
    dh = torch.empty(B, N, Fc, dtype=_H16[prec], device=dev)
    dg1 = torch.empty(B, N, 128, dtype=_H16[prec], device=dev)
    dg2 = torch.empty(B, N, 128, dtype=_H16[prec], device=dev)
    acc = {k: (sinks.get(k) if sinks.get(k) is not None else _zeros(arena, 128, device=dev)) for k in ('ln2_w', 'ln2_b', 'ln1_w', 'ln1_b')}
    dfilm = _zeros(arena, B, 256, device=dev) if film is not None else None
    datt = wt = None
    if out_pack is not None:
        if out_pack.cin != 128 or out_pack.cout != 128 or out_pack.taps != 1:
            raise ValueError('out_pack must be the (128, 128) out-projection')
        wt = out_pack.image(prec).bwd
        datt = torch.empty(B, N, 128, dtype=_H16[prec], device=dev)
    _log(pack1, ('ffpair', B * N, N, 128, Fc, 3))
    _fn('dx_ff_block_bwd', prec)(_p(dy2), _p(z2), _p(mean2), _p(rstd2), _p(ln2_w), _p(ln2_b), _p(film), 0 if film is None else film.stride(0),
                                 _p(dg2), _p(acc['ln2_w']), _p(acc['ln2_b']), _p(dfilm), 256, seed2, float(p2),
                                 _p(i2.bwd), _p(i1.bwd), _p(aux), _rows(aux), _p(dh), _rows(dh), _p(dz1), B, N, Fc, _p(lens), int(halo),
                                 _p(z1), _p(mean1), _p(rstd1), _p(ln1_w), _p(ln1_b), _p(dg1), _p(acc['ln1_w']), _p(acc['ln1_b']),
                                 seed1, float(p1), _p(wt), _p(datt), _p(seed_offset), _p(hmask), _stream())
    ret = lambda k: None if sinks.get(k) is not None else acc[k]
    return dz1, dh, dg1, dg2, dfilm, ret('ln2_w'), ret('ln2_b'), ret('ln1_w'), ret('ln1_b'), datt


class ZeroArena:

    def __init__(self, device, n_floats):
        self.buf = torch.zeros(int(n_floats), dtype=torch.float32, device=device)
        self.off = 0
        self.requested = 0

    @staticmethod
    def padded(n):
        return (int(n) + 3) // 4 * 4

    def take(self, *shape):
        n = 1
        for d in shape:
            n *= int(d)
        self.requested += self.padded(n)
        if self.off + n > self.buf.numel():
            return torch.zeros(*shape, dtype=torch.float32, device=self.buf.device)
        out = torch.empty(0, dtype=torch.float32, device=self.buf.device).set_(self.buf.untyped_storage(), self.off, tuple(int(d) for d in shape))
        self.off += self.padded(n)
        return out


def begin_step_arena(rt: Runtime, device) -> None:
    rt.arena = ZeroArena(device, rt.arena_hint)


def end_step_arena(rt: Runtime) -> None:
    if rt.arena is not None:
        rt.arena_hint = max(rt.arena_hint, int(1.25 * rt.arena.requested))
        rt.arena = None


def _zeros(arena, *shape, device=None):
    return arena.take(*shape) if arena is not None else torch.zeros(*shape, dtype=torch.float32, device=device)


def conv_wgrad(dy, x, pack: PackedWeight, lens=None, halo=-1, bias=True, arena=None, w_sink=None, b_sink=None, prec=None, defer=False):
    B_, N_ = (1, x.shape[0]) if x.dim() == 2 else (x.shape[0], x.shape[1])
    g = w_sink if w_sink is not None else _zeros(arena, *pack.weight.shape, device=x.device)
    db = b_sink if b_sink is not None else (_zeros(arena, pack.cout, device=x.device) if bias else None)
    _log(pack, ('wgrad', B_ * N_, N_, pack.cin, pack.cout, pack.taps))
    prec = prec or pack.rt.precision
    _check_h16(prec, dy, x)
    rt = pack.rt
    if (defer and rt.defer_wgrad and w_sink is not None and (b_sink is not None or not bias) and _half(prec) and pack.cin % 128 == 0
            and pack.cout % 8 == 0 and _rows(dy) % 8 == 0 and _rows(x) % 8 == 0):
        key = (pack.taps, _is_bf16(dy), _is_bf16(x), prec)
        rt.wgrad_queue.setdefault(key, []).append(((_p(dy), _p(x), _p(g), _p(db), _p(lens), _rows(dy), _rows(x), B_, N_, pack.cin, pack.cout,
                                                    int(halo), 0), (dy, x, g, db, lens)))
        return None, None
    _fn('dx_conv_wgrad', prec)(_p(dy), _rows(dy), _p(x), _rows(x), _p(g), B_, N_, pack.cin, pack.cout, pack.taps, _p(lens), int(halo),
                               _half(prec), _is_bf16(dy), _is_bf16(x), _p(db), _stream())
    return (None if w_sink is not None else g), (None if b_sink is not None else db)


class _WgradJob(ctypes.Structure):
    _fields_ = [(n, ctypes.c_void_p) for n in ('dY', 'X', 'G', 'dbias', 'lens')] + \
               [(n, ctypes.c_int) for n in ('ldy', 'ldx', 'B', 'N', 'Cin', 'Cout', 'skip_halo', 'reserved')]


WGRAD_BATCH = {1: 32, 3: 8}
WGRAD_BATCH_LOG = {}


def flush_wgrads(rt) -> int:
    launches = 0
    for (taps, dyh, xh, prec), jobs in rt.wgrad_queue.items():
        jobs.sort(key=lambda j: -j[0][7] * j[0][8])
        for i in range(0, len(jobs), WGRAD_BATCH[taps]):
            part = jobs[i:i + WGRAD_BATCH[taps]]
            arr = (_WgradJob * len(part))(*[_WgradJob(*fields) for fields, _ in part])
            if _lib.TIMER is not None:
                WGRAD_BATCH_LOG[ctypes.addressof(arr)] = (arr, [fields for fields, _ in part])
            _fn('dx_conv_wgrad_batched', prec)(ctypes.addressof(arr), len(part), taps, dyh, xh, _stream())
            launches += 1
    rt.wgrad_queue.clear()
    return launches


def film_affine_fwd(gammas, betas, pm, nb):
    B, total = gammas.shape
    C = total // nb
    film = torch.empty(nb, B, 2 * C, dtype=torch.float32, device=gammas.device)
    lib().dx_film_affine_fwd(_p(gammas), _p(betas), _p(pm), _p(film), B, nb, C, _stream())
    return film


def film_affine_bwd(dfilms, gammas, betas, pm, arena=None):
    B, total = gammas.shape
    nb = len(dfilms)
    C = total // nb
    dfilms = [None if g is None else g.contiguous() for g in dfilms]
    ptrs = (ctypes.c_void_p * nb)(*[None if g is None else g.data_ptr() for g in dfilms])
    dg, db = torch.empty_like(gammas), torch.empty_like(betas)
    dpm = _zeros(arena, 2, nb, device=gammas.device) if pm is not None else None
    lib().dx_film_affine_bwd(ctypes.addressof(ptrs), _p(gammas), _p(betas), _p(pm), _p(dg), _p(db), _p(dpm), B, nb, C, _stream())
    return dg, db, dpm


def colsum(x, C=None):
    C = x.shape[-1] if C is None else C
    rows = x.numel() // x.shape[-1]
    out = torch.zeros(C, dtype=torch.float32, device=x.device)
    lib().dx_colsum(_p(x), _rows(x), _p(out), rows, C, _is_bf16(x), _stream())
    return out




def length_order(lens_i32):
    order = torch.empty_like(lens_i32)
    lib().dx_length_order(_p(lens_i32), _p(order), lens_i32.shape[0], _stream())
    return order


def attention_fwd(qkv, lens, heads, seed, p_drop, prec=None, seed_offset=None, ctx_dtype=torch.float32, order=None):
    B, N, D3 = qkv.shape
    D = D3 // 3
    ctx = torch.empty(B, N, D, dtype=ctx_dtype, device=qkv.device)
    lse = torch.empty(B, heads, N, dtype=torch.float32, device=qkv.device)
    prec = prec or DEFAULT.precision
    _check_h16(prec, qkv, ctx)
    _fn('dx_attention_fwd', prec)(_p(qkv), _rows(qkv), _p(lens), _p(ctx), D, _p(lse), B, N, heads, D, seed, _p(seed_offset), float(p_drop),
                           _half(prec), _is_bf16(qkv), _is_bf16(ctx), _p(order), _stream())
    return ctx, lse


def attention_bwd(qkv, ctx, dctx, lse, lens, heads, seed, p_drop, out_dtype=torch.float32, prec=None, seed_offset=None, order=None):
    B, N, D3 = qkv.shape
    D = D3 // 3
    if dctx.dtype != ctx.dtype:
        raise TypeError(f'ctx ({ctx.dtype}) and dctx ({dctx.dtype}) must be stored alike')
    dqkv = torch.empty(B, N, D3, dtype=out_dtype, device=qkv.device)
    delta = torch.empty(B, heads, N, dtype=torch.float32, device=qkv.device)
    prec = prec or DEFAULT.precision
    _fn('dx_attention_bwd', prec)(_p(qkv), _rows(qkv), _p(ctx), _p(dctx), _rows(dctx), _p(lse), _p(delta), _p(lens), _p(dqkv), _rows(dqkv),
                           B, N, heads, D, seed, _p(seed_offset), float(p_drop), _half(prec), _is_bf16(qkv), _is_bf16(dqkv), _is_bf16(ctx),
                           _p(order), _stream())
    return dqkv


def gemm_shadow(prec=None):
    return bool(_half(prec or DEFAULT.precision))


def ln_fwd(a, res, w, b, film, lens, *, seed_pre=0, p_pre=0.0, seed_post=0, p_post=0.0, halo=0, shadow=False, seed_offset=None, prec=None):
    B, N, C = a.shape
    y = torch.empty_like(a)
    prec = prec or DEFAULT.precision
    y_h = torch.empty(B, N, C, dtype=_H16[prec], device=a.device) if shadow else None
    mean = torch.empty(B, N, dtype=torch.float32, device=a.device)
    rstd = torch.empty(B, N, dtype=torch.float32, device=a.device)
    _fn('dx_ln_fwd', prec)(_p(a), _p(res), _p(w), _p(b), _p(film), 0 if film is None else film.stride(0), _p(lens), int(halo), _p(y), _p(mean), _p(rstd),
                    B, N, C, seed_pre, float(p_pre), seed_post, float(p_post), _p(seed_offset), _is_bf16(a), _p(y_h), _stream())
    return (y, mean, rstd, y_h) if shadow else (y, mean, rstd)


def attn_proj_ln_applies(qkv, heads, pack: PackedWeight, prec) -> bool:
    return (prec in _H16 and qkv.dtype == _H16[prec] and qkv.dim() == 3 and qkv.shape[2] == 384 and heads == 2
            and pack.taps == 1 and pack.cin == 128 and pack.cout == 128)


def attn_proj_ln_fwd(qkv, lens, heads, seed, p_drop, pack: PackedWeight, proj_bias, res, w, b, film, *, seed_pre=0, p_pre=0.0, shadow=False,
                     seed_offset=None, prec=None):
    B, N, D3 = qkv.shape
    D = D3 // 3
    prec = prec or pack.rt.precision
    _check_h16(prec, qkv)
    h16 = _H16[prec]
    ctx = torch.empty(B, N, D, dtype=h16, device=qkv.device)
    lse = torch.empty(B, heads, N, dtype=torch.float32, device=qkv.device)
    z = torch.empty(B, N, D, dtype=torch.float32, device=qkv.device)
    y = torch.empty_like(z)
    y_h = torch.empty(B, N, D, dtype=h16, device=qkv.device) if shadow else None
    mean = torch.empty(B, N, dtype=torch.float32, device=qkv.device)
    rstd = torch.empty(B, N, dtype=torch.float32, device=qkv.device)
    img = pack.image(prec)
    _log(pack, ('gemm', B * N, N, pack.cin, pack.cout, 1))
    _fn('dx_attention_proj_ln_fwd', prec)(_p(qkv), _rows(qkv), _p(lens), _p(ctx), D, _p(lse), B, N, heads, D, seed, _p(seed_offset), float(p_drop),
                                          _p(img.fwd), _p(proj_bias), _p(z), _p(res), _p(w), _p(b), _p(film), 0 if film is None else film.stride(0),
                                          _p(y), _p(mean), _p(rstd), seed_pre, float(p_pre), _p(y_h), _stream())
    return (ctx, lse, z, y, mean, rstd, y_h) if shadow else (ctx, lse, z, y, mean, rstd)


def proj_ln_fwd(x, pack: PackedWeight, proj_bias, res, w, b, film, lens, *, seed_pre=0, p_pre=0.0, halo=0, shadow=False, seed_offset=None, prec=None):
    B, N, C = x.shape
    prec = prec or pack.rt.precision
    _check_h16(prec, x)
    img = pack.image(prec)
    z = torch.empty(B, N, C, dtype=torch.float32, device=x.device)
    y = torch.empty_like(z)
    y_h = torch.empty(B, N, C, dtype=_H16[prec], device=x.device) if shadow else None
    mean = torch.empty(B, N, dtype=torch.float32, device=x.device)
    rstd = torch.empty(B, N, dtype=torch.float32, device=x.device)
    _log(pack, ('gemm', B * N, N, pack.cin, pack.cout, 1))
    _fn('dx_proj_ln_fwd', prec)(_p(x), _rows(x), _p(img.fwd), _p(proj_bias), _p(z), _p(res), _p(w), _p(b), _p(film), 0 if film is None else film.stride(0),
                                _p(lens), int(halo), _p(y), _p(mean), _p(rstd), B, N, seed_pre, float(p_pre), _p(seed_offset), _p(y_h), _stream())
    return (z, y, mean, rstd, y_h) if shadow else (z, y, mean, rstd)


def ln_bwd(dy, z, mean, rstd, w, b, film, lens, *, relu_mask=False, want_da=False, seed_pre=0, p_pre=0.0, seed_post=0, p_post=0.0,
           arena=None, w_sink=None, b_sink=None, halo=0, shadow=False, seed_offset=None, prec=None):
    B, N, C = z.shape
    dz = torch.empty_like(z)
    prec = prec or DEFAULT.precision
    dg_h = torch.empty(B, N, C, dtype=_H16[prec], device=z.device) if shadow else None
    da = torch.empty_like(z) if (want_da and not shadow) else None
    dw = w_sink if w_sink is not None else _zeros(arena, C, device=z.device)
    db = b_sink if b_sink is not None else _zeros(arena, C, device=z.device)
    dfilm = _zeros(arena, B, 2 * C, device=z.device) if film is not None else None
    _fn('dx_ln_bwd', prec)(_p(dy), _p(z), _p(mean), _p(rstd), _p(w), _p(b), _p(film), 0 if film is None else film.stride(0), _p(lens), int(halo),
                    _p(dz), _p(da), _p(dw), _p(db), _p(dfilm), 2 * C, B, N, C, int(relu_mask),
                    seed_pre, float(p_pre), seed_post, float(p_post), _p(seed_offset), _is_bf16(z), _p(dg_h), _stream())
    out = (dz, da, (None if w_sink is not None else dw), (None if b_sink is not None else db), dfilm)
    return out + (dg_h,) if shadow else out


def add_pos(x, sym, emb, pe, lens):
    if emb is not None:
        B, N = sym.shape
        D = emb.shape[1]
    else:
        B, N, D = x.shape
    out = torch.empty(B, N, D, dtype=torch.float32, device=pe.device)
    lib().dx_add_pos(_p(x), _p(sym), _p(emb), _p(pe), _p(lens), _p(out), B, N, D, pe.shape[0], _stream())
    return out


def mask_rows(x, lens):
    B, N, C = x.shape
    out = torch.empty_like(x)
    lib().dx_mask_rows(_p(x), _p(lens), _p(out), B, N, C, _stream())
    return out


def embedding_bwd(dout, sym, lens, n_rows, arena=None, sink=None):
    B, N, D = dout.shape
    demb = sink if sink is not None else _zeros(arena, n_rows, D, device=dout.device)
    lib().dx_embedding_bwd(_p(dout), _p(sym), _p(lens), _p(demb), B, N, D, _stream())
    return None if sink is not None else demb


def accent_sum(prenet, energy, pitch, we, be, wp, bp, pe, lens):
    B, N, D = prenet.shape
    out = torch.empty_like(prenet)
    lib().dx_accent_sum(_p(prenet), _p(energy), _p(pitch), _p(we), _p(be), _p(wp), _p(bp), _p(pe), _p(lens), _p(out), B, N, D, pe.shape[0], _stream())
    return out


def scalar_conv_wgrad(dout, s0, s1, lens, rowscale=None, sinks=None):
    B, N = s0.shape
    D = 128
    dev = s0.device
    sinks = sinks or (None, None, None, None)
    dw0 = sinks[0] if sinks[0] is not None else torch.zeros(D, 1, 3, dtype=torch.float32, device=dev)
    db0 = sinks[1] if sinks[1] is not None else torch.zeros(D, dtype=torch.float32, device=dev)
    dw1 = (sinks[2] if sinks[2] is not None else torch.zeros(D, 1, 3, dtype=torch.float32, device=dev)) if s1 is not None else None
    db1 = (sinks[3] if sinks[3] is not None else torch.zeros(D, dtype=torch.float32, device=dev)) if s1 is not None else None
    ldd = dout.stride(-2) if dout.dim() == 3 else 0
    lib().dx_scalar_conv_wgrad(_p(dout), ldd, _p(rowscale), _p(s0), _p(s1), _p(lens), _p(dw0), _p(db0), _p(dw1), _p(db1), B, N, D, _stream())
    return tuple(None if sk is not None else t for sk, t in zip(sinks, (dw0, db0, dw1, db1)))


def mean_pool(x, lens, arena=None):
    B, N, C = x.shape
    out = _zeros(arena, B, C, device=x.device)
    lib().dx_mean_pool(_p(x), _p(lens), _p(out), B, N, C, _stream())
    return out


def mean_pool_bwd(dout, lens, N):
    B, C = dout.shape
    dx = torch.empty(B, N, C, dtype=torch.float32, device=dout.device)
    lib().dx_mean_pool_bwd(_p(dout), _p(lens), _p(dx), B, N, C, _stream())
    return dx


def transpose(x, add_to=None):
    B, R, C = x.shape
    out = add_to if add_to is not None else torch.empty(B, C, R, dtype=torch.float32, device=x.device)
    lib().dx_transpose(_p(x), _p(out), B, R, C, int(add_to is not None), _stream())
    return out


def l2_normalize(x):
    y = torch.empty_like(x)
    lib().dx_l2_normalize(_p(x), _p(y), x.shape[0], x.shape[1], _stream())
    return y


def cross_entropy(logits, target):
    B, S = logits.shape
    loss = torch.empty(1, dtype=torch.float32, device=logits.device)
    dlogits = torch.empty_like(logits)
    lib().dx_cross_entropy(_p(logits), _p(target), _p(loss), _p(dlogits), B, S, _stream())
    return loss, dlogits


def duration_scan(dur_int):
    B, L = dur_int.shape
    mu = torch.empty(B, L, dtype=torch.float32, device=dur_int.device)
    totals = torch.empty(B, dtype=torch.long, device=dur_int.device)
    lib().dx_duration_scan(_p(dur_int), _p(mu), _p(totals), B, L, _stream())
    return mu, totals


def upsample_prep(enc, dur, energy, pitch, wd, bd, we, be, wp, bp, wr, br, lens):
    B, L, D = enc.shape
    xs = torch.empty_like(enc)
    z = torch.empty(B, L, dtype=torch.float32, device=enc.device)
    sigma = torch.empty(B, L, dtype=torch.float32, device=enc.device)
    lib().dx_upsample_prep(_p(enc), _p(dur), _p(energy), _p(pitch), _p(wd), _p(bd), _p(we), _p(be), _p(wp), _p(bp), _p(wr), _p(br),
                           _p(lens), _p(xs), _p(z), _p(sigma), B, L, D, _stream())
    return xs, z, sigma


def upsample_fwd(xs, mu, sigma, lens, T):
    B, L, D = xs.shape
    weights = torch.empty(B, L, T, dtype=torch.float32, device=xs.device)
    xup = torch.empty(B, T, D, dtype=torch.float32, device=xs.device)
    lib().dx_upsample_fwd(_p(xs), _p(mu), _p(sigma), _p(lens), _p(weights), _p(xup), B, L, T, D, _stream())
    return xup, weights


def upsample_bwd(dxup, xs, mu, sigma, weights, lens, arena=None):
    B, L, D = xs.shape
    T = weights.shape[2]
    dxs = _zeros(arena, B, L, D, device=xs.device)
    dsigma = _zeros(arena, B, L, device=xs.device)
    lib().dx_upsample_bwd(_p(dxup), _p(xs), _p(mu), _p(sigma), _p(weights), _p(lens), _p(dxs), _p(dsigma), B, L, T, D, _stream())
    return dxs, dsigma


def upsample_sym_bwd(dxs, dsigma, xs, z, dur, lens, wd, bd, wr, dwr_sink=None, dbr_sink=None):
    B, L, D = xs.shape
    dxs_out = torch.empty_like(xs)
    dz = torch.empty(B, L, dtype=torch.float32, device=xs.device)
    dwr = dwr_sink if dwr_sink is not None else torch.zeros(D, dtype=torch.float32, device=xs.device)
    dbr = dbr_sink if dbr_sink is not None else torch.zeros(1, dtype=torch.float32, device=xs.device)
    lib().dx_upsample_sym_bwd(_p(dxs), _p(dsigma), _p(xs), _p(z), _p(dur), _p(lens), _p(wd), _p(bd), _p(wr), _p(dxs_out), _p(dz), _p(dwr), _p(dbr),
                              B, L, D, _stream())
    return dxs_out, dz, (None if dwr_sink is not None else dwr), (None if dbr_sink is not None else dbr)


def mel_stats(mel_pred, mel_target, arena=None):
    B, M, T = mel_pred.shape
    dev = mel_pred.device
    ep = torch.empty(B, T, dtype=torch.float32, device=dev)
    et = torch.empty(B, T, dtype=torch.float32, device=dev)
    sums = _zeros(arena, 2, B, device=dev)
    lib().dx_mel_stats(_p(mel_pred), _p(mel_target), _p(ep), _p(et), _p(sums[0]), _p(sums[1]), B, M, T, _stream())
    return ep, et, sums


def energy_diff(ep, et, lens, arena=None):
    B, T = ep.shape
    des = torch.empty_like(ep)
    esum = _zeros(arena, 1, device=ep.device)
    lib().dx_energy_diff(_p(ep), _p(et), _p(lens), _p(des), _p(esum), B, T, _stream())
    return des, esum


def mel_grad(mel_pred, mel_target, ep, des, lens, c_l1, c_l2, c_e, e_per_total=False):
    B, M, T = mel_pred.shape
    dmel = torch.empty_like(mel_pred)
    lib().dx_mel_grad(_p(mel_pred), _p(mel_target), _p(ep), _p(des), _p(lens), float(c_l1), float(c_l2), float(c_e), int(e_per_total), _p(dmel),
                      B, M, T, _stream())
    return dmel


def loss_finalize(ce, dlogits, spk_w, pm, pmw, sums, lens, M, msw, esum, ecw, psum, pcw, grad_scale=1.0):
    dev = sums.device
    B = sums.shape[1]
    out = torch.empty(8, dtype=torch.float32, device=dev)
    d_spk = torch.empty_like(dlogits) if dlogits is not None else None
    d_pm = torch.empty_like(pm) if pm is not None else None
    w_dev = spk_w if torch.is_tensor(spk_w) else None
    lib().dx_loss_finalize(_p(ce), _p(w_dev), 0.0 if w_dev is not None else float(spk_w), _p(dlogits), _p(d_spk), 0 if dlogits is None else dlogits.numel(),
                           _p(pm), _p(d_pm), 0 if pm is None else pm.numel(), float(pmw), _p(sums[0]), _p(sums[1]), _p(lens), B, M, float(msw),
                           _p(esum), float(ecw), _p(psum), float(pcw), _p(out), _p(out[7:]), float(grad_scale), _stream())
    return out[:7], out[7], d_spk, d_pm


def _frame_stride(t):
    return 1 if t.dim() == 2 else t.shape[2]


def pitch_mse(pp, gt, lens, arena=None):
    B, T = gt.shape
    sums = _zeros(arena, 2, device=gt.device)
    lib().dx_pitch_mse(_p(pp), _frame_stride(pp), _p(gt), _p(lens), _p(sums), B, T, _stream())
    return sums


def pitch_grad(pp, gt, lens, sums, scale, out=None):
    B, T = gt.shape
    dpp = out if out is not None else torch.empty(B, T, dtype=torch.float32, device=gt.device)
    lib().dx_pitch_grad(_p(pp), _frame_stride(pp), _p(gt), _p(lens), _p(sums), float(scale), _p(dpp), _frame_stride(dpp), B, T, _stream())
    return dpp


def pitch_chain_applies(layers, mel, prec) -> bool:
    if not _half(prec) or len(layers) != 4 or mel.dim() != 3 or not (64 < mel.shape[1] <= 96) or mel.shape[0] > 1000:
        return False
    shapes = [tuple(l['pack'].weight.shape) for l in layers]
    M = mel.shape[1]
    return (shapes[0] == (256, M, 3) and shapes[1] == (256, 256, 3) and shapes[2] == (256, 256, 3) and shapes[3][1:] == (256, 3)
            and all(l['scale'] is not None for l in layers[:3]))


def pitch_chain_fwd(mel, layers, lens, prec, arena=None):
    B, M, T = mel.shape
    pp = _zeros(arena, B, T, device=mel.device)
    masks = torch.empty(B, T, 3, 8, dtype=torch.int32, device=mel.device)
    img = [l['pack'].image(prec) for l in layers[:3]]
    _fn('dx_pitch_chain_fwd', prec)(_p(mel), B, M, T, _p(lens), _p(img[0].fwd), _p(img[1].fwd), _p(img[2].fwd),
                                    _p(layers[0]['b']), _p(layers[1]['b']), _p(layers[2]['b']),
                                    _p(layers[0]['scale']), _p(layers[1]['scale']), _p(layers[2]['scale']),
                                    _p(layers[0]['shift']), _p(layers[1]['shift']), _p(layers[2]['shift']),
                                    _p(layers[3]['w']), float(layers[3]['b3']), _p(pp), _p(masks), _stream())
    return pp, masks


def pitch_chain_bwd(dpp, masks, layers, lens, prec, dmel):
    B, M, T = dmel.shape
    img = [l['pack'].image(prec) for l in layers[:3]]
    _fn('dx_pitch_chain_bwd', prec)(_p(dpp), B, M, T, _p(lens), _p(img[0].bwd), _p(img[1].bwd), _p(img[2].bwd),
                                    _p(layers[0]['scale']), _p(layers[1]['scale']), _p(layers[2]['scale']),
                                    _p(layers[3]['w']), _p(masks), _p(dmel), _stream())
    return dmel


def relu_bwd(dy, y):
    out = torch.empty_like(dy)
    lib().dx_relu_bwd(_p(dy), _p(y), _p(out), dy.numel(), _stream())
    return out


def channel_affine(x, scale, shift, prec=None):
    out = torch.empty_like(x)
    fn = _fn('dx_channel_affine', prec or DEFAULT.precision) if _is_bf16(x) else lib().dx_channel_affine
    fn(_p(x), _p(scale), _p(shift), _p(out), x.numel() // x.shape[-1], x.shape[-1], _is_bf16(x), _stream())
    return out
```

Measured before the change: 4.793 million.

## Split FF-pair hidden dimension across blocks with ticketed slab reduction for small grids

```diff
diff --git a/include/daft_exprt_hip.h b/include/daft_exprt_hip.h
--- a/include/daft_exprt_hip.h
+++ b/include/daft_exprt_hip.h
@@ -36,25 +36,28 @@
 int dx_unpack_wgrad(const float* G, float* grad, int Cout, int Cin, int taps, int accumulate, void* stream);
 int dx_ff_pair(const void* X, int ldx, const void* Wa, const void* Wb, const float* bias_a, const float* bias_b,
                const void* aux, int ld_aux, void* H, int ldh, float* Y, int ldy,
-               int B, int N, int F, int relu_mid, int accumulate, const int* lens, int skip_halo, const int* rows_exist, void* stream);
+               int B, int N, int F, int relu_mid, int accumulate, const int* lens, int skip_halo, const int* rows_exist, void* workspace, void* stream);
+int dx_ff_pair_workspace_size(int B, int N, int F, long* bytes);
 int dx_ff_pair_ln(const void* X, int ldx, const void* Wa, const void* Wb, const float* bias_a, const float* bias_b, void* H, int ldh, float* Z,
                   int B, int N, int F, const int* lens, int skip_halo, const int* rows_exist,
                   const float* res, const float* ln_w, const float* ln_b, const float* film, int ld_film, float* Yln, float* mean, float* rstd,
-                  uint64_t seed_pre, float p_pre, const uint64_t* seed_offset, void* hmask, void* stream);
+                  uint64_t seed_pre, float p_pre, const uint64_t* seed_offset, void* hmask, void* workspace, void* stream);
 int dx_ff_pair_ln_qkv(const void* X, int ldx, const void* Wa, const void* Wb, const float* bias_a, const float* bias_b, void* H, int ldh, float* Z,
                       int B, int N, int F, const int* lens, int skip_halo, const int* rows_exist,
                       const float* res, const float* ln_w, const float* ln_b, const float* film, int ld_film, float* Yln, float* mean, float* rstd,
-                      uint64_t seed_pre, float p_pre, const uint64_t* seed_offset, const void* Wq, const float* bias_q, void* QKV, void* hmask, void* stream);
+                      uint64_t seed_pre, float p_pre, const uint64_t* seed_offset, const void* Wq, const float* bias_q, void* QKV, void* hmask,
+                      void* workspace, void* stream);
 int dx_ff_pair_lnbwd(const void* X, int ldx, const void* Wa, const void* Wb, const void* aux, int ld_aux, void* H, int ldh, float* Y,
                      int B, int N, int F, const int* lens, int skip_halo,
                      const float* z, const float* mean, const float* rstd, const float* ln_w, const float* ln_b, void* DG, float* dw, float* db,
-                     uint64_t seed_pre, float p_pre, const uint64_t* seed_offset, void* stream);
+                     uint64_t seed_pre, float p_pre, const uint64_t* seed_offset, void* workspace, void* stream);
 int dx_ff_block_bwd(const float* dY2, const float* z2, const float* mean2, const float* rstd2, const float* ln2_w, const float* ln2_b,
                     const float* film, int ld_film, void* DG2, float* dw2, float* db2, float* dfilm, int ld_dfilm, uint64_t seed2, float p2,
                     const void* Wa, const void* Wb, const void* aux, int ld_aux, void* H, int ldh, float* Y,
                     int B, int N, int F, const int* lens, int skip_halo,
                     const float* z1, const float* mean1, const float* rstd1, const float* ln1_w, const float* ln1_b, void* DG1, float* dw1, float* db1,
-                    uint64_t seed1, float p1, const void* Wout_bwd, void* DATT, const uint64_t* seed_offset, const void* hmask, void* stream);
+                    uint64_t seed1, float p1, const void* Wout_bwd, void* DATT, const uint64_t* seed_offset, const void* hmask, void* workspace,
+                    void* stream);
 int dx_colsum(const void* X, int ldx, float* out, long rows, int C, int x_bf16, void* stream);
 
 int dx_length_order(const int* lens, int* order, int B, void* stream);
diff --git a/ubisoft_laforge_daft_exprt_amd/csrc/dx_f16_names.h b/ubisoft_laforge_daft_exprt_amd/csrc/dx_f16_names.h
--- a/ubisoft_laforge_daft_exprt_amd/csrc/dx_f16_names.h
+++ b/ubisoft_laforge_daft_exprt_amd/csrc/dx_f16_names.h
@@ -17,6 +17,7 @@
 #define dx_ff_pair_ln dx_ff_pair_ln_f16
 #define dx_ff_pair_ln_qkv dx_ff_pair_ln_qkv_f16
 #define dx_ff_pair_lnbwd dx_ff_pair_lnbwd_f16
+#define dx_ff_pair_workspace_size dx_ff_pair_workspace_size_f16
 #define dx_gather_speaker_rows dx_gather_speaker_rows_f16
 #define dx_l2_normalize dx_l2_normalize_f16
 #define dx_length_order dx_length_order_f16
diff --git a/ubisoft_laforge_daft_exprt_amd/csrc/dx_ffpair.hip b/ubisoft_laforge_daft_exprt_amd/csrc/dx_ffpair.hip
--- a/ubisoft_laforge_daft_exprt_amd/csrc/dx_ffpair.hip
+++ b/ubisoft_laforge_daft_exprt_amd/csrc/dx_ffpair.hip
@@ -37,6 +37,7 @@
   unsigned long long lnp_seed; unsigned lnp_thresh; float lnp_inv_keep;
   unsigned* hmask;
   unsigned long long* stamps;
+  int nsplit; float* slab; unsigned* tickets;
 };
 
 #ifdef DX_FFPAIR_STAMPS
@@ -82,14 +83,27 @@
   const int tiles_n = (a.N + FP_TOK - 1) / FP_TOK;
   const int nslices = a.F >> 7;
   FP_STAMP(0)
-
-  const dx_h16* const wbase = role == 0 ? a.Wa + (size_t)(2 * wq) * 4 * 512
-                                        : a.Wb + (size_t)(2 * wq) * (a.F >> 5) * 512;
+  constexpr bool SPLIT = NJ == 4;
+  int tile_id = blockIdx.x, split = 0, fs0 = 0, nsl = nslices;
+  if constexpr (SPLIT) {
+    if (a.nsplit > 1) {
+      const int S = a.nsplit, chunk = blockIdx.x / (8 * S), w8 = blockIdx.x - chunk * 8 * S;
+      split = w8 >> 3;
+      tile_id = chunk * 8 + (w8 & 7);
+      if (tile_id >= a.B * tiles_n) return;
+      const int q = nslices / S, rem = nslices - q * S;
+      fs0 = split * q + min(split, rem);
+      nsl = q + (split < rem ? 1 : 0);
+    }
+  }
+
+  const dx_h16* const wbase = role == 0 ? a.Wa + (size_t)(2 * wq) * 4 * 512 + (size_t)fs0 * (8 * 4 * 512)
+                                        : a.Wb + (size_t)(2 * wq) * (a.F >> 5) * 512 + (size_t)fs0 * (4 * 512);
   const unsigned lane16 = lane * 16;
   const int w_tap = role == 0 ? (a.F >> 4) * 4 * 512 : 8 * (a.F >> 5) * 512;
   const int w_i = role == 0 ? 4 * 512 : (a.F >> 5) * 512;
   const int w_slice = role == 0 ? 8 * 4 * 512 : 4 * 512;
-  const int total_steps = nslices * 12;
+  const int total_steps = nsl * 12;
   auto w_ptr = [&](int gs) {
     gs = min(gs, total_steps - 1);
     const int f = fp_opaque(gs / 12), s = gs - f * 12;
@@ -118,7 +132,7 @@
       if (base == 0) { cnt0 = cnt; inc0 = inc; }
       nlive += __shfl(inc, 63, 64);
     }
-    int target = blockIdx.x;
+    int target = tile_id;
     live = target < nlive;
     if (!live) target -= nlive;
     int run = 0;
@@ -147,14 +161,15 @@
       run += __shfl(inc, 63, 64);
     }
   } else {
-    b = blockIdx.x / tiles_n;
-    n0 = (blockIdx.x - b * tiles_n) * FP_TOK;
+    b = (unsigned)tile_id / tiles_n;
+    n0 = ((unsigned)tile_id - b * tiles_n) * FP_TOK;
   }
   FP_STAMP(1)
   b = __builtin_amdgcn_readfirstlane(b);
   n0 = __builtin_amdgcn_readfirstlane(n0);
 
   if (!live) {
+    if (split != 0) return;
     const int rows = min(FP_TOK, a.N - n0);
     const int hu = a.H ? a.F >> 3 : 0;
     for (int u = tid; u < rows * hu; u += 512) {
@@ -264,7 +279,7 @@
 #pragma unroll
       for (int e = 0; e < 8; ++e) h8[e] = (dx_h16)dz[e];
       const f32x4 hv = __builtin_bit_cast(f32x4, h8);
-      if (owned) *reinterpret_cast<f32x4*>(a.lnp_dg + grow * 128 + q * 8) = hv;
+      if (owned && split == 0) *reinterpret_cast<f32x4*>(a.lnp_dg + grow * 128 + q * 8) = hv;
       if (row < FP_HR) *reinterpret_cast<f32x4*>(Xs + (q >> 3) * (FP_HR * 128) + fp_lds_off(row, q & 7)) = hv;
     }
 #pragma unroll
@@ -289,7 +304,7 @@
       float t = 0.f;
 #pragma unroll
       for (int w8 = 0; w8 < 8; ++w8) t += red[(w8 * 4 + quant) * 128 + c];
-      if (t != 0.f) {
+      if (t != 0.f && split == 0) {
         if (quant == 0) atomicAdd(&a.lnp_dw[c], t);
         else if (quant == 1) atomicAdd(&a.lnp_db[c], t);
         else if (a.lnp_dfilm) atomicAdd(&a.lnp_dfilm[(size_t)b * a.lnp_ld_dfilm + (quant == 3 ? 128 : 0) + c], t);
@@ -406,7 +421,7 @@
     const int tile_lin = b * tiles_n + n0 / FP_TOK;
 #define FP_PRODUCE(F_, COFLAG)                                                                                       \
     {                                                                                                                \
-      const int f0 = (F_) << 7;                                                                                      \
+      const int f0 = (fs0 + (F_)) << 7;                                                                              \
                                    \
       const f32x4 bv0 = a.bias_a ? *reinterpret_cast<const f32x4*>(a.bias_a + f0 + 32 * wq + 4 * g) : f32x4{0.f, 0.f, 0.f, 0.f};      \
       const f32x4 bv1 = a.bias_a ? *reinterpret_cast<const f32x4*>(a.bias_a + f0 + 32 * wq + 16 + 4 * g) : f32x4{0.f, 0.f, 0.f, 0.f}; \
@@ -426,7 +441,7 @@
               av[i][j] = *reinterpret_cast<const bf16x4*>(a.aux + ((size_t)b * a.N + n) * a.ld_aux + f0 + 32 * wq + 16 * i + 4 * g2_); \
             }                                                                                                        \
           }                                                                                                          \
-        }, true, COFLAG, ((((F_) - 1) & 1) ? Hs1 : Hs0), ((F_) - 1) * 128)                                           \
+        }, true, COFLAG, ((((F_) - 1) & 1) ? Hs1 : Hs0), (fs0 + (F_) - 1) * 128)                                     \
       unsigned char* const out = ((F_) & 1) ? Hs1 : Hs0;                                                             \
       const int r_ = fp_opaque(r);                                                                                   \
       const int g_ = fp_opaque(g);                                                                                   \
@@ -475,7 +490,7 @@
     FP_PRODUCE(0, false)
     __syncthreads();
     FP_STAMP(3)
-    for (int it = 1; it < nslices; ++it) {
+    for (int it = 1; it < nsl; ++it) {
       if (it == 4) FP_STAMP(12)
       FP_PRODUCE(it, true)
       if (it == 4) FP_STAMP(14)
@@ -483,13 +498,13 @@
       FP_STAMP(3 + it)
     }
     {
-      const unsigned char* const imgc = ((nslices - 1) & 1) ? Hs1 : Hs0;
+      const unsigned char* const imgc = ((nsl - 1) & 1) ? Hs1 : Hs0;
       f32x4 cpv;
 #pragma unroll
-      for (int k = 0; k < NJ / 2; ++k) { FP_CO_RD(k, imgc) FP_CO_ST(k, (nslices - 1) << 7) }
+      for (int k = 0; k < NJ / 2; ++k) { FP_CO_RD(k, imgc) FP_CO_ST(k, (fs0 + nsl - 1) << 7) }
     }
     __syncthreads();
-    FP_STAMP(3 + nslices)
+    FP_STAMP(3 + nsl)
 #undef FP_PRODUCE
   } else {
     f32x4 acc[2][NJ];
@@ -500,24 +515,39 @@
       for (int j = 0; j < NJ; ++j) acc[i][j] = f32x4{0.f, 0.f, 0.f, 0.f};
     __syncthreads();
     FP_STAMP(3)
-    for (int it = 1; it <= nslices; ++it) {
+    for (int it = 1; it <= nsl; ++it) {
       if (it == 4) FP_STAMP(12)
       const int f = it - 1;
       const unsigned char* const img = (f & 1) ? Hs1 : Hs0;
-      FP_COPY_OUT_CONS(img, f << 7)
+      FP_COPY_OUT_CONS(img, (fs0 + f) << 7)
       FP_SLICE_STEPS(img, f * 12, , false, false, img, 0)
       if (it == 4) FP_STAMP(13)
       __syncthreads();
       FP_STAMP(3 + it)
     }
-#pragma unroll
-    for (int i = 0; i < 2; ++i) {
-      const int co = 32 * wq + 16 * i + 4 * g;
-      const f32x4 bv = a.bias_b ? *reinterpret_cast<const f32x4*>(a.bias_b + co) : f32x4{0.f, 0.f, 0.f, 0.f};
-#pragma unroll
-      for (int j = 0; j < NJ; ++j) {
-        const int q = 16 * j + r;
-        *reinterpret_cast<f32x4*>(stage + q * 512 + (((co >> 2) ^ (q & 15)) << 4)) = acc[i][j] + bv;
+    bool to_stage = true;
+    if constexpr (SPLIT) {
+      if (a.nsplit > 1) {
+        f32x4* const sl = reinterpret_cast<f32x4*>(a.slab) + ((size_t)tile_id * a.nsplit + split) * (8 * NJ * 64);
+#pragma unroll
+        for (int i = 0; i < 2; ++i)
+#pragma unroll
+          for (int j = 0; j < NJ; ++j)
+            asm volatile("global_store_dwordx4 %0, %1, off sc1\n\ts_nop 1" :: "v"(sl + ((wq * 2 + i) * NJ + j) * 64 + lane), "v"(acc[i][j]) : "memory");
+        asm volatile("s_waitcnt vmcnt(0)" ::: "memory");
+        to_stage = false;
+      }
+    }
+    if (to_stage) {
+#pragma unroll
+      for (int i = 0; i < 2; ++i) {
+        const int co = 32 * wq + 16 * i + 4 * g;
+        const f32x4 bv = a.bias_b ? *reinterpret_cast<const f32x4*>(a.bias_b + co) : f32x4{0.f, 0.f, 0.f, 0.f};
+#pragma unroll
+        for (int j = 0; j < NJ; ++j) {
+          const int q = 16 * j + r;
+          *reinterpret_cast<f32x4*>(stage + q * 512 + (((co >> 2) ^ (q & 15)) << 4)) = acc[i][j] + bv;
+        }
       }
     }
   }
@@ -529,6 +559,44 @@
 #undef FP_CO_ST
 
   __syncthreads();
+  if constexpr (SPLIT) {
+    if (a.nsplit > 1) {
+      int* const last_flag = reinterpret_cast<int*>(smem + 2 * FP_IMG);
+      if (tid == 0) {
+        const unsigned ticket = __hip_atomic_fetch_add(a.tickets + tile_id, 1u, __ATOMIC_RELAXED, __HIP_MEMORY_SCOPE_AGENT);
+        const int last = ticket == (unsigned)(a.nsplit - 1);
+        if (last) {
+          __builtin_amdgcn_fence(__ATOMIC_ACQUIRE, "agent");
+          asm volatile("s_waitcnt vmcnt(0)" ::: "memory");
+          __hip_atomic_store(a.tickets + tile_id, 0u, __ATOMIC_RELAXED, __HIP_MEMORY_SCOPE_AGENT);
+        }
+        *last_flag = last;
+      }
+      __syncthreads();
+      if (!*last_flag) return;
+      constexpr int FR = 8 * NJ * 64;
+      const f32x4* const sl = reinterpret_cast<const f32x4*>(a.slab) + (size_t)tile_id * a.nsplit * FR;
+      f32x4 v[FR / 512], v1[FR / 512];
+#pragma unroll
+      for (int k = 0; k < FR / 512; ++k) { v[k] = sl[tid + k * 512]; v1[k] = sl[FR + tid + k * 512]; }
+#pragma unroll
+      for (int k = 0; k < FR / 512; ++k) v[k] += v1[k];
+      for (int s = 2; s < a.nsplit; ++s) {
+#pragma unroll
+        for (int k = 0; k < FR / 512; ++k) v1[k] = sl[(size_t)s * FR + tid + k * 512];
+#pragma unroll
+        for (int k = 0; k < FR / 512; ++k) v[k] += v1[k];
+      }
+#pragma unroll
+      for (int k = 0; k < FR / 512; ++k) {
+        const int u = tid + k * 512, ln = u & 63, j = (u >> 6) % NJ, i = ((u >> 6) / NJ) & 1, wq2 = (u >> 6) / NJ >> 1;
+        const int co = 32 * wq2 + 16 * i + 4 * (ln >> 4), q = 16 * j + (ln & 15);
+        const f32x4 bv = a.bias_b ? *reinterpret_cast<const f32x4*>(a.bias_b + co) : f32x4{0.f, 0.f, 0.f, 0.f};
+        *reinterpret_cast<f32x4*>(stage + q * 512 + (((co >> 2) ^ (q & 15)) << 4)) = v[k] + bv;
+      }
+      __syncthreads();
+    }
+  }
   if (a.ln_w) {
     const int s = tid & 31;
     const f32x4 wv = *reinterpret_cast<const f32x4*>(a.ln_w + s * 4), bv = *reinterpret_cast<const f32x4*>(a.ln_b + s * 4);
@@ -744,7 +812,25 @@
 extern "C" void dx_ff_pair_set_stamps(unsigned long long* p) { g_ffpair_stamps = p; }
 #endif
 
+static int ff_pair_nj(int B, int N) { return B * dx_cdiv(N, FP<8>::TOK) >= 96 ? 8 : 4; }
+
+static int ff_pair_nsplit(int B, int N, int F) {
+  if (ff_pair_nj(B, N) == 8) return 1;
+  return (F >> 7) >= 2 && 2 * B * dx_cdiv(N, FP<4>::TOK) <= 256 ? 2 : 1;
+}
+constexpr size_t FF_TICKET_BYTES = 128 * 4;
+static size_t ff_pair_workspace_bytes(int B, int N, int F) {
+  const int S = ff_pair_nsplit(B, N, F), tiles = B * dx_cdiv(N, FP<4>::TOK);
+  return S > 1 ? FF_TICKET_BYTES + (size_t)tiles * S * (8 * 4 * 64) * sizeof(f32x4) : 0;
+}
+
 extern "C" {
+
+int dx_ff_pair_workspace_size(int B, int N, int F, long* bytes) {
+  DX_REQUIRE(bytes && B > 0 && N > 0 && F >= 128 && (F % 128) == 0, "dx_ff_pair_workspace_size: bad arguments");
+  *bytes = (long)ff_pair_workspace_bytes(B, N, F);
+  return DX_OK;
+}
 
 static int ff_pair_launch(const void* X, int ldx, const void* Wa, const void* Wb, const float* bias_a, const float* bias_b,
                           const void* aux, int ld_aux, void* H, int ldh, float* Y, int ldy,
@@ -752,7 +838,7 @@
                           const float* ln_res, const float* ln_w, const float* ln_b, const float* film, int ld_film,
                           float* ln_y, float* ln_mean, float* ln_rstd, unsigned long long seed_pre, float p_pre, const unsigned long long* seed_offset,
                           const float* lnb_z, const float* lnb_mean, const float* lnb_rstd, const float* lnb_w, const float* lnb_b,
-                          void* lnb_dg, float* lnb_dw, float* lnb_db, const FFPairArgs* prologue, void* stream, unsigned* hmask = nullptr) {
+                          void* lnb_dg, float* lnb_dw, float* lnb_db, const FFPairArgs* prologue, void* workspace, void* stream, unsigned* hmask = nullptr) {
   DX_REQUIRE((X || prologue) && Wa && Wb && Y, "dx_ff_pair: null pointer");
   DX_REQUIRE(H || (relu_mid && !lnb_w), "dx_ff_pair: only the forward pair may omit the mid-activation output H");
   if (ln_w) {
@@ -812,17 +898,27 @@
     configured = true;
   }
   a.hmask = hmask;
-  const int nj = B * dx_cdiv(N, FP<8>::TOK) >= 96 ? 8 : 4;
+  const int nj = ff_pair_nj(B, N);
+  const int tiles4 = B * dx_cdiv(N, FP<4>::TOK);
+  a.nsplit = ff_pair_nsplit(B, N, F);
   hipStream_t s = (hipStream_t)stream;
+  if (a.nsplit > 1) {
+    DX_REQUIRE(workspace && ((uintptr_t)workspace % 256) == 0, "dx_ff_pair: this shape splits the hidden dimension and needs a 256-byte aligned, "
+               "zero-initialised workspace of dx_ff_pair_workspace_size() bytes");
+    DX_REQUIRE((size_t)tiles4 * 4 <= FF_TICKET_BYTES, "dx_ff_pair: %d tiles do not fit the ticket block", tiles4);
+    a.tickets = (unsigned*)workspace;
+    a.slab = (float*)((char*)workspace + FF_TICKET_BYTES);
+  }
   dx_prof_begin(DX_PROF_CONV_GEMM, s);
   if (nj == 8) {
     if (aux && hmask) hipLaunchKernelGGL((ff_pair_kernel<true, false, 8, true>), dim3(B * dx_cdiv(N, FP<8>::TOK)), dim3(512), lds8, s, a);
     else if (aux) hipLaunchKernelGGL((ff_pair_kernel<true, false, 8>), dim3(B * dx_cdiv(N, FP<8>::TOK)), dim3(512), lds8, s, a);
     else hipLaunchKernelGGL((ff_pair_kernel<false, true, 8>), dim3(B * dx_cdiv(N, FP<8>::TOK)), dim3(512), 3 * FP<8>::IMG, s, a);
   } else {
-    if (aux && hmask) hipLaunchKernelGGL((ff_pair_kernel<true, false, 4, true>), dim3(B * dx_cdiv(N, FP<4>::TOK)), dim3(512), lds4, s, a);
-    else if (aux) hipLaunchKernelGGL((ff_pair_kernel<true, false, 4>), dim3(B * dx_cdiv(N, FP<4>::TOK)), dim3(512), lds4, s, a);
-    else hipLaunchKernelGGL((ff_pair_kernel<false, true, 4>), dim3(B * dx_cdiv(N, FP<4>::TOK)), dim3(512), 3 * FP<4>::IMG, s, a);
+    const int grid4 = a.nsplit > 1 ? dx_cdiv(tiles4, 8) * 8 * a.nsplit : tiles4;
+    if (aux && hmask) hipLaunchKernelGGL((ff_pair_kernel<true, false, 4, true>), dim3(grid4), dim3(512), lds4, s, a);
+    else if (aux) hipLaunchKernelGGL((ff_pair_kernel<true, false, 4>), dim3(grid4), dim3(512), lds4, s, a);
+    else hipLaunchKernelGGL((ff_pair_kernel<false, true, 4>), dim3(grid4), dim3(512), 3 * FP<4>::IMG, s, a);
   }
   dx_prof_end(DX_PROF_CONV_GEMM, s);
   DX_LAUNCH_CHECK("dx_ff_pair");
@@ -831,42 +927,43 @@
 
 int dx_ff_pair(const void* X, int ldx, const void* Wa, const void* Wb, const float* bias_a, const float* bias_b,
                const void* aux, int ld_aux, void* H, int ldh, float* Y, int ldy,
-               int B, int N, int F, int relu_mid, int accumulate, const int* lens, int skip_halo, const int* rows_exist, void* stream) {
+               int B, int N, int F, int relu_mid, int accumulate, const int* lens, int skip_halo, const int* rows_exist, void* workspace, void* stream) {
   return ff_pair_launch(X, ldx, Wa, Wb, bias_a, bias_b, aux, ld_aux, H, ldh, Y, ldy, B, N, F, relu_mid, accumulate, lens, skip_halo, rows_exist,
                         nullptr, nullptr, nullptr, nullptr, 0, nullptr, nullptr, nullptr, 0ull, 0.f, nullptr,
-                        nullptr, nullptr, nullptr, nullptr, nullptr, nullptr, nullptr, nullptr, nullptr, stream);
+                        nullptr, nullptr, nullptr, nullptr, nullptr, nullptr, nullptr, nullptr, nullptr, workspace, stream);
 }
 
 int dx_ff_pair_ln(const void* X, int ldx, const void* Wa, const void* Wb, const float* bias_a, const float* bias_b, void* H, int ldh, float* Z,
                   int B, int N, int F, const int* lens, int skip_halo, const int* rows_exist,
                   const float* res, const float* ln_w, const float* ln_b, const float* film, int ld_film, float* Yln, float* mean, float* rstd,
-                  uint64_t seed_pre, float p_pre, const uint64_t* seed_offset, void* hmask, void* stream) {
+                  uint64_t seed_pre, float p_pre, const uint64_t* seed_offset, void* hmask, void* workspace, void* stream) {
   DX_REQUIRE(ln_w != nullptr, "dx_ff_pair_ln: null pointer");
   return ff_pair_launch(X, ldx, Wa, Wb, bias_a, bias_b, nullptr, 0, H, ldh, Z, 128, B, N, F, 1, 0, lens, skip_halo, rows_exist,
                         res, ln_w, ln_b, film, ld_film, Yln, mean, rstd, (unsigned long long)seed_pre, p_pre, (const unsigned long long*)seed_offset,
-                        nullptr, nullptr, nullptr, nullptr, nullptr, nullptr, nullptr, nullptr, nullptr, stream, (unsigned*)hmask);
+                        nullptr, nullptr, nullptr, nullptr, nullptr, nullptr, nullptr, nullptr, nullptr, workspace, stream, (unsigned*)hmask);
 }
 
 int dx_ff_pair_ln_qkv(const void* X, int ldx, const void* Wa, const void* Wb, const float* bias_a, const float* bias_b, void* H, int ldh, float* Z,
                       int B, int N, int F, const int* lens, int skip_halo, const int* rows_exist,
                       const float* res, const float* ln_w, const float* ln_b, const float* film, int ld_film, float* Yln, float* mean, float* rstd,
-                      uint64_t seed_pre, float p_pre, const uint64_t* seed_offset, const void* Wq, const float* bias_q, void* QKV, void* hmask, void* stream) {
+                      uint64_t seed_pre, float p_pre, const uint64_t* seed_offset, const void* Wq, const float* bias_q, void* QKV, void* hmask,
+                      void* workspace, void* stream) {
   DX_REQUIRE(ln_w != nullptr && Wq != nullptr, "dx_ff_pair_ln_qkv: null pointer");
   FFPairArgs ext{};
   ext.q_w = (const dx_h16*)Wq; ext.q_bias = bias_q; ext.q_out = (dx_h16*)QKV;
   return ff_pair_launch(X, ldx, Wa, Wb, bias_a, bias_b, nullptr, 0, H, ldh, Z, 128, B, N, F, 1, 0, lens, skip_halo, rows_exist,
                         res, ln_w, ln_b, film, ld_film, Yln, mean, rstd, (unsigned long long)seed_pre, p_pre, (const unsigned long long*)seed_offset,
-                        nullptr, nullptr, nullptr, nullptr, nullptr, nullptr, nullptr, nullptr, &ext, stream, (unsigned*)hmask);
+                        nullptr, nullptr, nullptr, nullptr, nullptr, nullptr, nullptr, nullptr, &ext, workspace, stream, (unsigned*)hmask);
 }
 
 int dx_ff_pair_lnbwd(const void* X, int ldx, const void* Wa, const void* Wb, const void* aux, int ld_aux, void* H, int ldh, float* Y,
                      int B, int N, int F, const int* lens, int skip_halo,
                      const float* z, const float* mean, const float* rstd, const float* ln_w, const float* ln_b, void* DG, float* dw, float* db,
-                     uint64_t seed_pre, float p_pre, const uint64_t* seed_offset, void* stream) {
+                     uint64_t seed_pre, float p_pre, const uint64_t* seed_offset, void* workspace, void* stream) {
   DX_REQUIRE(ln_w != nullptr, "dx_ff_pair_lnbwd: null pointer");
   return ff_pair_launch(X, ldx, Wa, Wb, nullptr, nullptr, aux, ld_aux, H, ldh, Y, 128, B, N, F, 0, 1, lens, skip_halo, nullptr,
                         nullptr, nullptr, nullptr, nullptr, 0, nullptr, nullptr, nullptr, (unsigned long long)seed_pre, p_pre, (const unsigned long long*)seed_offset,
-                        z, mean, rstd, ln_w, ln_b, DG, dw, db, nullptr, stream);
+                        z, mean, rstd, ln_w, ln_b, DG, dw, db, nullptr, workspace, stream);
 }
 
 int dx_ff_block_bwd(const float* dY2, const float* z2, const float* mean2, const float* rstd2, const float* ln2_w, const float* ln2_b,
@@ -874,7 +971,8 @@
                     const void* Wa, const void* Wb, const void* aux, int ld_aux, void* H, int ldh, float* Y,
                     int B, int N, int F, const int* lens, int skip_halo,
                     const float* z1, const float* mean1, const float* rstd1, const float* ln1_w, const float* ln1_b, void* DG1, float* dw1, float* db1,
-                    uint64_t seed1, float p1, const void* Wout_bwd, void* DATT, const uint64_t* seed_offset, const void* hmask, void* stream) {
+                    uint64_t seed1, float p1, const void* Wout_bwd, void* DATT, const uint64_t* seed_offset, const void* hmask, void* workspace,
+                    void* stream) {
   DX_REQUIRE(ln1_w != nullptr && ln2_w != nullptr, "dx_ff_block_bwd: null pointer");
   DX_REQUIRE((Wout_bwd == nullptr) == (DATT == nullptr) && ((uintptr_t)Wout_bwd % 16) == 0 && ((uintptr_t)DATT % 16) == 0, "dx_ff_block_bwd: Wout_bwd and DATT come together, 16-byte aligned");
   DX_REQUIRE(p2 >= 0.f && p2 < 1.f, "dx_ff_block_bwd: dropout p out of range");
@@ -886,7 +984,7 @@
   pro.lnp_ld_dfilm = ld_dfilm; pro.lnp_seed = (unsigned long long)seed2; pro.lnp_thresh = (unsigned)lrintf(p2 * 65536.f); pro.lnp_inv_keep = 1.f / (1.f - p2);
   return ff_pair_launch(nullptr, 128, Wa, Wb, nullptr, nullptr, aux, ld_aux, H, ldh, Y, 128, B, N, F, 0, 1, lens, skip_halo, nullptr,
                         nullptr, nullptr, nullptr, nullptr, 0, nullptr, nullptr, nullptr, (unsigned long long)seed1, p1, (const unsigned long long*)seed_offset,
-                        z1, mean1, rstd1, ln1_w, ln1_b, DG1, dw1, db1, &pro, stream, (unsigned*)hmask);
-}
-
-}
+                        z1, mean1, rstd1, ln1_w, ln1_b, DG1, dw1, db1, &pro, workspace, stream, (unsigned*)hmask);
+}
+
+}
diff --git a/ubisoft_laforge_daft_exprt_amd/ops.py b/ubisoft_laforge_daft_exprt_amd/ops.py
--- a/ubisoft_laforge_daft_exprt_amd/ops.py
+++ b/ubisoft_laforge_daft_exprt_amd/ops.py
@@ -250,6 +250,24 @@
             and (x.shape[0] * ((x.shape[1] + 125) // 126) >= _FF_FUSED_MIN_TILES or x.shape[0] * ((x.shape[1] + 61) // 62) >= _FF_FUSED_MIN_TILES62))
 
 
+_FF_WS = {}
+_FF_WS_RETIRED = []
+
+
+def _ff_workspace(B, N, Fc, prec, device):
+    need = ctypes.c_long(0)
+    _fn('dx_ff_pair_workspace_size', prec)(B, N, Fc, ctypes.addressof(need))
+    if need.value == 0:
+        return None
+    key = (device, _stream(), torch.cuda.is_current_stream_capturing())
+    ws = _FF_WS.get(key)
+    if ws is None or ws.numel() < need.value:
+        if ws is not None:
+            _FF_WS_RETIRED.append(ws)
+        ws = _FF_WS[key] = torch.zeros(need.value, dtype=torch.uint8, device=device)
+    return ws
+
+
 def ff_pair(x, pack1: PackedWeight, pack2: PackedWeight, bias1, bias2, lens, *, backward=False, aux=None, out=None, accumulate=False,
             halo=1, prec=None, rows_exist=None):
     prec = pack1.rt.precision if prec is None else prec
@@ -266,7 +284,8 @@
         out = torch.empty(B, N, 128, dtype=torch.float32, device=x.device)
     _log(pack1, ('ffpair', B * N, N, 128, Fc, 3))
     _fn('dx_ff_pair', prec)(_p(x), _rows(x), _p(wa), _p(wb), _p(bias1), _p(bias2), _p(aux), 0 if aux is None else _rows(aux), _p(h), _rows(h),
-                     _p(out), _rows(out), B, N, Fc, int(not backward), int(accumulate), _p(lens), int(halo), _p(rows_exist), _stream())
+                     _p(out), _rows(out), B, N, Fc, int(not backward), int(accumulate), _p(lens), int(halo), _p(rows_exist),
+                     _p(_ff_workspace(B, N, Fc, prec, x.device)), _stream())
     return out, h
 
 
@@ -288,17 +307,18 @@
     mask = torch.empty(B * ((N + 61) // 62), Fc // 128, 4, 2, 64, dtype=torch.int32, device=x.device) if want_mask else None
     tail = (mask,) if want_mask else ()
     _log(pack1, ('ffpair', B * N, N, 128, Fc, 3))
+    ws = _ff_workspace(B, N, Fc, prec, x.device)
     if next_in is not None:
         pq, bq = next_in
         qkv = torch.empty(B, N, 384, dtype=_H16[prec], device=x.device)
         _log(pq, ('conv', B * N, N, 128, 384, 1))
         _fn('dx_ff_pair_ln_qkv', prec)(_p(x), _rows(x), _p(i1.fwd), _p(i2.fwd), _p(bias1), _p(bias2), _p(h), Fc if h is None else _rows(h), _p(z), B, N, Fc, _p(lens), int(halo),
                                        _p(rows_exist), _p(res), _p(ln_w), _p(ln_b), _p(film), 0 if film is None else film.stride(0), _p(y), _p(mean),
-                                       _p(rstd), seed_pre, float(p_pre), _p(seed_offset), _p(pq.image(prec).fwd), _p(bq), _p(qkv), _p(mask), _stream())
+                                       _p(rstd), seed_pre, float(p_pre), _p(seed_offset), _p(pq.image(prec).fwd), _p(bq), _p(qkv), _p(mask), _p(ws), _stream())
         return (z, h, y, mean, rstd, qkv) + tail
     _fn('dx_ff_pair_ln', prec)(_p(x), _rows(x), _p(i1.fwd), _p(i2.fwd), _p(bias1), _p(bias2), _p(h), Fc if h is None else _rows(h), _p(z), B, N, Fc, _p(lens), int(halo),
                                _p(rows_exist), _p(res), _p(ln_w), _p(ln_b), _p(film), 0 if film is None else film.stride(0), _p(y), _p(mean), _p(rstd),
-                               seed_pre, float(p_pre), _p(seed_offset), _p(mask), _stream())
+                               seed_pre, float(p_pre), _p(seed_offset), _p(mask), _p(ws), _stream())
     return (z, h, y, mean, rstd) + tail
 
 
@@ -316,7 +336,8 @@
     db = b_sink if b_sink is not None else _zeros(arena, 128, device=x.device)
     _log(pack1, ('ffpair', B * N, N, 128, Fc, 3))
     _fn('dx_ff_pair_lnbwd', prec)(_p(x), _rows(x), _p(i2.bwd), _p(i1.bwd), _p(aux), _rows(aux), _p(dh), _rows(dh), _p(out), B, N, Fc, _p(lens), int(halo),
-                                  _p(z), _p(mean), _p(rstd), _p(ln_w), _p(ln_b), _p(dg), _p(dw), _p(db), seed_pre, float(p_pre), _p(seed_offset), _stream())
+                                  _p(z), _p(mean), _p(rstd), _p(ln_w), _p(ln_b), _p(dg), _p(dw), _p(db), seed_pre, float(p_pre), _p(seed_offset),
+                                  _p(_ff_workspace(B, N, Fc, prec, x.device)), _stream())
     return out, dh, dg, (None if w_sink is not None else dw), (None if b_sink is not None else db)
 
 
@@ -345,7 +366,7 @@
                                  _p(dg2), _p(acc['ln2_w']), _p(acc['ln2_b']), _p(dfilm), 256, seed2, float(p2),
                                  _p(i2.bwd), _p(i1.bwd), _p(aux), _rows(aux), _p(dh), _rows(dh), _p(dz1), B, N, Fc, _p(lens), int(halo),
                                  _p(z1), _p(mean1), _p(rstd1), _p(ln1_w), _p(ln1_b), _p(dg1), _p(acc['ln1_w']), _p(acc['ln1_b']),
-                                 seed1, float(p1), _p(wt), _p(datt), _p(seed_offset), _p(hmask), _stream())
+                                 seed1, float(p1), _p(wt), _p(datt), _p(seed_offset), _p(hmask), _p(_ff_workspace(B, N, Fc, prec, dev)), _stream())
     ret = lambda k: None if sinks.get(k) is not None else acc[k]
     return dz1, dh, dg1, dg2, dfilm, ret('ln2_w'), ret('ln2_b'), ret('ln1_w'), ret('ln1_b'), datt
 
```

Result: faster. 4.844 million, median of 6 (+1.1%).
